# ZhengyiLuo/PHC

Hardware: AMD Instinct MI355X
Metric: env-steps/sec at 4096 humanoid envs per GPU (VecEnv.step incl. resets) (higher is better)
Workload: dtype f32

## Files before the change

### include/phc_amd.h

```cpp
#ifndef PHC_AMD_H
#define PHC_AMD_H
#include <stdint.h>

#ifdef __cplusplus
extern "C" {
#endif

#define PHC_ABI_VERSION 37
#define PHC_MAX_BODIES 64
#define PHC_EINVAL (-1)
#define PHC_EUNSUPPORTED (-2)
#define PHC_RESET_SUBLISTS 16
#define PHC_RESET_COUNT_STRIDE 32

typedef struct {
    int32_t num_bodies;
    int32_t num_dof;
    int32_t max_level;
    int32_t num_contact_pts;
    const int32_t* ints;
    const float* floats;
    int32_t num_collision_pairs;
    int32_t num_shapes;
    int32_t int_stride;
    int32_t float_stride;
    int32_t max_body_contact_pts;
} phc_model_t;

typedef struct {
    const float* frames;
    int64_t num_frames_total;
    int32_t frame_stride;
    int32_t num_bodies;
    int32_t num_motions;
    const float* motion_lengths;
    const float* motion_dt;
    const int64_t* motion_num_frames;
    const int64_t* length_starts;
    int32_t num_ext_bodies;
    int32_t dofs_per_joint;
} phc_motion_lib_t;

typedef struct {
    int32_t num_envs;
    float* root_states;
    float* dof_state;
    float* rigid_body_state;
    float* contact_force;
    float* dof_force;
    float* pd_target;
    float* force_sensor;
    const int32_t* env_shape;
    const float* pd_ref;
} phc_sim_state_t;

typedef struct {
    float sim_dt;
    int32_t substeps;
    int32_t control_freq_inv;
    float gravity_z;
    float contact_stiffness;
    float contact_damping;
    float friction;
    float friction_viscous;
    float angular_damping;
    float max_angular_velocity;
    float contact_offset;
    int32_t control_mode;
    float limit_stiffness;
    float limit_damping;
    int32_t self_collision;
    float self_stiffness_scale;
    float self_damping_ratio;
    int32_t lane_mapping;
    int32_t num_force_sensors;
    int32_t force_sensor_body[4];
    int32_t contact_model;
    int32_t contact_iterations;
    float contact_impedance;
    float max_depenetration_velocity;
    float bounce_threshold_velocity;
    float restitution;
    int32_t inertia_lag;
    int32_t force_average;
} phc_sim_params_t;

typedef struct {
    float dt;
    int32_t max_episode_length;
    float k_pos, k_rot, k_vel, k_ang_vel, w_pos, w_rot, w_vel, w_ang_vel;
    int32_t power_reward;
    float power_coefficient;
    int32_t enable_early_termination;
    int32_t use_mean_termination;
    int32_t disable_collision_check;
    int32_t local_root_obs, root_height_obs;
    int32_t num_track_bodies;
    const int32_t* track_slot;
    const int32_t* reset_mask;
    int32_t num_reset_bodies;
    int32_t first_reset_body;
    const float* termination_distances;
    int32_t num_key_bodies;
    const int32_t* key_body_ids;
    int32_t num_amp_joints;
    const int32_t* amp_joint_slot;
    int32_t num_amp_obs_steps;
    int32_t num_amp_obs_per_step;
    int32_t num_self_obs, num_task_obs;
    int32_t cycle_motion;
    int32_t zero_out_far;
    float close_distance;
    float far_distance;
    int32_t dofs_per_joint;
    int32_t num_ext_bodies;
    const int32_t* ext_parent;
    const float* ext_offset;
    int32_t obs_v;
    int32_t self_obs_v;
    int32_t num_force_sensors;
    int32_t amp_obs_v;
    int32_t remove_base_rot;
    int32_t num_self_obs_extra;
    int32_t num_amp_obs_extra;
    int32_t num_traj_samples;
    float traj_sample_timestep;
    int32_t track_body_reward;
    int32_t num_self_obs_hist;
    int32_t zero_out_far_train;
    int32_t zero_out_far_steps;
    int32_t cycle_motion_xp;
    const float* self_obs_extra;
    const float* amp_obs_extra;
    const float* amp_ref_table;
} phc_im_params_t;

typedef struct {
    int64_t* progress_buf;
    int64_t* reset_buf;
    int64_t* terminate_buf;
    float* rew_buf;
    float* reward_raw;
    float* obs_buf;
    float* amp_obs_in;
    float* amp_obs_out;
    const int64_t* sampled_motion_ids;
    float* motion_start_times;
    float* motion_start_times_offset;
    float* global_offset;
    float* ref_body_pos;
    float* ref_body_rot;
    float* ref_body_vel;
    float* ref_dof_pos;
    int32_t* cycle_counter;
    int32_t* recovery_counter;
    float* point_goal;
    const float* cycle_phase;
    int32_t* reset_list;
    int32_t* reset_count;
    int32_t reset_slot;
    int32_t reset_sublist_cap;
    float* body_state_hist;
    const float* offset_rand;
    const uint8_t* occl_mask;
    int64_t amp_env_stride;
    uint64_t* reset_rng_counter;
} phc_im_buffers_t;

int32_t phc_abi_version(void);

int32_t phc_motion_state(const phc_motion_lib_t* lib, int32_t n, const int64_t* motion_ids, const float* motion_times,
                         const float* offset, float* rg_pos , float* rb_rot ,
                         float* body_vel , float* body_ang_vel , float* dof_pos ,
                         float* dof_vel , int64_t* frame_idx0 , int64_t* frame_idx1 ,
                         float* blend , float* rg_pos_ext , float* rb_rot_ext , void* stream);

int32_t phc_sample_time_interval(const phc_motion_lib_t* lib, int32_t n, const int64_t* motion_ids, const float* phase,
                                 float* motion_times, void* stream);

int32_t phc_sim_step(const phc_model_t* model, const phc_sim_params_t* params, const phc_sim_state_t* sim,
                     const float* actions , const float* pd_action_offset , const float* pd_action_scale ,
                     const int32_t* freeze_mask , int32_t num_sim_calls, void* stream);

int32_t phc_sim_step_wrench(const phc_model_t* model, const phc_sim_params_t* params, const phc_sim_state_t* sim,
                            const float* actions , const float* pd_action_offset , const float* pd_action_scale ,
                            const int32_t* freeze_mask , int32_t num_sim_calls,
                            const float* ext_force , const float* ext_torque , int32_t wrench_sim_calls, void* stream);

int32_t phc_refresh_body_state(const phc_model_t* model, const phc_sim_state_t* sim, void* stream);

int32_t phc_refresh_body_state_indexed(const phc_model_t* model, const phc_sim_state_t* sim, int32_t num, const int64_t* env_ids,
                                       void* stream);

int32_t phc_im_post_physics(const phc_model_t* model, const phc_motion_lib_t* lib, const phc_im_params_t* prm,
                            const phc_sim_state_t* sim, const phc_im_buffers_t* buf, void* stream);

int32_t phc_amp_ref_table(const phc_model_t* model, const phc_motion_lib_t* lib, const phc_im_params_t* prm, int64_t num_frames,
                          const int64_t* next_frame , float* table , void* stream);

int32_t phc_im_reset(const phc_model_t* model, const phc_motion_lib_t* lib, const phc_im_params_t* prm,
                     const phc_sim_state_t* sim, const phc_im_buffers_t* buf, int32_t num_reset,
                     const int64_t* env_ids, const float* phase , int32_t start_at_zero, void* stream);

int32_t phc_im_is_plain(const phc_model_t* model, const phc_motion_lib_t* lib, const phc_im_params_t* prm, const phc_im_buffers_t* buf);
int32_t phc_task_force_generic(int32_t on);

int32_t phc_im_reset_done(const phc_model_t* model, const phc_motion_lib_t* lib, const phc_im_params_t* prm,
                          const phc_sim_state_t* sim, const phc_im_buffers_t* buf, uint64_t seed, uint64_t counter,
                          int32_t start_at_zero, void* stream);

int32_t phc_im_reset_from_state(const phc_model_t* model, const phc_motion_lib_t* lib, const phc_im_params_t* prm,
                                const phc_sim_state_t* sim, const phc_im_buffers_t* buf, int32_t num_reset,
                                const int64_t* env_ids, int32_t fill_history, void* stream);

int32_t phc_amp_obs_demo(const phc_model_t* model, const phc_motion_lib_t* lib, const phc_im_params_t* prm, int32_t n,
                         const int64_t* motion_ids, const float* motion_times0, float* amp_obs_demo , void* stream);

int32_t phc_gae(int32_t horizon, int32_t n, const float* fdones, const float* values, const float* rewards,
                const float* next_values, float gamma, float tau, float* advs, void* stream);

int32_t phc_fk(const phc_model_t* model, int64_t num_frames, const float* local_rot, const float* root_trans,
               float* global_rot, float* global_pos, void* stream);

int64_t phc_running_norm_workspace(int64_t rows, int32_t cols);
int32_t phc_running_norm(const float* x, const int64_t* row_index, int64_t rows, int32_t cols, const double* norm_mean, const double* norm_var, float epsilon,
                         float clamp, void* out, int32_t out_bf16, int32_t out_stride, double* run_mean, double* run_var, double* run_count,
                         double* workspace, void* stream);

int64_t phc_colsum_workspace(int64_t rows, int32_t cols);
int32_t phc_colsum_bf16(const void* x, int64_t rows, int32_t cols, float* out, float* workspace, void* stream);
int32_t phc_colsum_relu_bf16(const void* gy, const void* y, int64_t rows, int32_t cols, void* gm, float* out, float* workspace, void* stream);
#define PHC_COLSUM_MAX_JOBS 16
typedef struct {
    const float* partial;
    float* out;
    int32_t nchunks, cols, accumulate;
} phc_colsum_job_t;
int32_t phc_colsum_chunks(int64_t rows);
int32_t phc_linear1_chunks(int64_t rows);
int32_t phc_colsum_finish_batch(int32_t count, const phc_colsum_job_t* jobs , void* stream);
int32_t phc_sum_slabs_bf16(const void* part, int32_t slabs, int64_t n, float* out, int32_t accumulate, void* stream);
int32_t phc_split3_bf16(const float* x, int64_t ld_in, const float* gate, int64_t ld_gate, int64_t rows, int32_t cols, int64_t rows_pad, int32_t cols_pad,
                        const float* extra, int32_t extra_mode, void* out, int64_t row_stride, int64_t chunk_stride, int32_t order, void* stream);

int32_t phc_wgrad_bf16_slices(int64_t rows, int32_t n, int32_t k);
int64_t phc_wgrad_bf16_workspace(int64_t rows, int32_t n, int32_t k);
int32_t phc_wgrad_bf16(const void* gy, const void* y, const void* x, int64_t ld_x, int64_t rows, int32_t n, int32_t k, float* gw, int64_t ld_gw,
                       int32_t accumulate, void* gz, float* gb, int32_t gb_accumulate, void* workspace, void* stream);

int32_t phc_disc_bce(const void* logits, int32_t is_bf16, int32_t n_agent, int32_t n_demo, float scale, void* grad, float* stats,
                     void* stream);
int64_t phc_sumsq_workspace(void);
int32_t phc_weighted_sumsq(int32_t count, const void* const* tensors, const int64_t* sizes, const float* coefs, int32_t is_bf16, float* out,
                           double* workspace, void* stream);

int32_t phc_rollout_bookkeeping(const float* rewards, float reward_scale, const int64_t* dones, const int64_t* terminate, const float* reward_raw,
                                int32_t num_reward_terms, int64_t num_envs, float* exp_rewards, uint8_t* exp_dones, float* terminated_flags,
                                float* terminated_mask, float* reward_raw_acc, float* current_rewards, float* current_lengths, void* stream);

int32_t phc_policy_sample(const void* mu, const void* value, int32_t is_bf16, const float* logstd, const float* noise, const double* value_mean,
                          const double* value_var, float epsilon, const float* mask, int64_t num_envs, int32_t num_actions, float* actions, float* mus,
                          float* sigmas, float* neglogp, float* values, void* stream);

int64_t phc_linear1_workspace(int64_t rows, int32_t cols);
int32_t phc_linear1_forward(const void* x, const void* w, const void* b, int64_t rows, int32_t cols, void* y, void* stream);
int32_t phc_linear1_backward(const void* x, const void* w, const void* gy, int64_t rows, int32_t cols, void* gx, float* gw_gb,
                             float* workspace, void* stream);

int64_t phc_adam_workspace(void);
int32_t phc_adam_clip_step(float* param, float* grad, float* exp_avg, float* exp_avg_sq, int64_t n, float lr, float beta1, float beta2,
                           float eps, float weight_decay, int64_t step, float max_norm, double* workspace, float* grad_norm_out,
                           void* param_bf16, int64_t* step_device, void* stream);

typedef struct {
    float e_clip, critic_coef, entropy_coef, bounds_loss_coef;
    int32_t clip_value;
} phc_ppo_params_t;
int64_t phc_ppo_loss_workspace(void);
int32_t phc_ppo_loss(const void* mu, const void* value, int32_t is_bf16, const float* logstd, const float* actions, const float* old_neglogp,
                     const float* advantages, const float* returns, const float* old_values, const float* old_mu, const float* old_sigma,
                     const int64_t* row_index, int64_t batch, int32_t num_actions, const phc_ppo_params_t* prm, void* grad_mu, void* grad_value, float* stats,
                     double* workspace, void* stream);

#define PHC_RENDER_MAX_PIXELS (1 << 24)
#define PHC_RENDER_MAX_SHAPES 128
#define PHC_RENDER_MAX_MARKERS 128
#define PHC_RENDER_PALETTE 16
#define PHC_RENDER_MARKER_ID 1000
typedef struct {
    int32_t env;
    float eye[3], target[3], up[3];
    float fov_y;
} phc_camera_t;
typedef struct {
    int32_t num_envs, num_bodies;
    const float* body_state;
    const float* capsules;
    int32_t num_capsules;
    int32_t num_shape_blocks;
    int64_t capsule_stride;
    const int32_t* env_shape;
    const float* markers;
    int32_t num_markers;
    float marker_radius;
    float palette[PHC_RENDER_PALETTE][3];
    float marker_color[3];
    float ground_color[2][3];
    float sky_color[3];
    float light_dir[3];
    float ambient, diffuse;
} phc_render_scene_t;
int32_t phc_render(const phc_render_scene_t* scene , const phc_camera_t* cameras , int32_t views, int32_t width,
                   int32_t height, uint8_t* rgba, float* depth, int32_t* hit_id, void* stream);

typedef struct {
    int32_t num_envs, num_bodies;
    int32_t root_idx;
    int32_t step;
    int32_t bound;
    float dt;
    const float* rigid_body_state;
    const int64_t* progress_buf;
    const int64_t* terminate_buf;
    const int64_t* motion_ids;
    const float* motion_start_times;
    const float* motion_start_times_offset;
    const float* global_offset;
    const int32_t* clip_steps;
    float* history;
    double* sums;
    int32_t* count;
    int32_t* failed;
    int32_t* status;
    float* mpjpe_step;
    float* gt_out;
} phc_eval_args_t;
int32_t phc_eval_accumulate(const phc_motion_lib_t* lib, const phc_eval_args_t* args , void* stream);

typedef struct {
    int32_t num_envs, num_bodies;
    int32_t num_listed;
    int32_t pause_lo, pause_hi;
    int32_t duration;
    int32_t direction;
    float force_lo, force_hi;
    uint64_t key;
    int64_t env_offset;
    const int32_t* bodies;
    const int64_t* progress_buf;
    int32_t* remaining;
    int32_t* countdown;
    int32_t* body;
    int32_t* k;
    int32_t* started;
    float* force;
} phc_push_args_t;
int32_t phc_push_advance(const phc_push_args_t* args , void* stream);

#ifdef __cplusplus
}
#endif
#endif
```

### phc_amd/_lib.py

```python
import ctypes as C
import os

import torch

HERE = os.path.dirname(os.path.abspath(__file__))
LIB_PATH = os.environ.get("PHC_AMD_LIB") or os.path.join(HERE, "libphc_amd.so")

c_f = C.c_float
c_i32 = C.c_int32
c_i64 = C.c_int64
c_p = C.c_void_p


class Model(C.Structure):
    _fields_ = [("num_bodies", c_i32), ("num_dof", c_i32), ("max_level", c_i32), ("num_contact_pts", c_i32),
                ("ints", c_p), ("floats", c_p), ("num_collision_pairs", c_i32),
                ("num_shapes", c_i32), ("int_stride", c_i32), ("float_stride", c_i32), ("max_body_contact_pts", c_i32)]


class MotionLib(C.Structure):
    _fields_ = [("frames", c_p), ("num_frames_total", c_i64), ("frame_stride", c_i32), ("num_bodies", c_i32),
                ("num_motions", c_i32), ("motion_lengths", c_p), ("motion_dt", c_p), ("motion_num_frames", c_p),
                ("length_starts", c_p), ("num_ext_bodies", c_i32), ("dofs_per_joint", c_i32)]


class SimState(C.Structure):
    _fields_ = [("num_envs", c_i32), ("root_states", c_p), ("dof_state", c_p), ("rigid_body_state", c_p),
                ("contact_force", c_p), ("dof_force", c_p), ("pd_target", c_p), ("force_sensor", c_p), ("env_shape", c_p), ("pd_ref", c_p)]


class SimParams(C.Structure):
    _fields_ = [("sim_dt", c_f), ("substeps", c_i32), ("control_freq_inv", c_i32), ("gravity_z", c_f),
                ("contact_stiffness", c_f), ("contact_damping", c_f), ("friction", c_f), ("friction_viscous", c_f),
                ("angular_damping", c_f), ("max_angular_velocity", c_f), ("contact_offset", c_f),
                ("control_mode", c_i32), ("limit_stiffness", c_f), ("limit_damping", c_f),
                ("self_collision", c_i32), ("self_stiffness_scale", c_f), ("self_damping_ratio", c_f), ("lane_mapping", c_i32),
                ("num_force_sensors", c_i32), ("force_sensor_body", c_i32 * 4),
                ("contact_model", c_i32), ("contact_iterations", c_i32), ("contact_impedance", c_f), ("max_depenetration_velocity", c_f),
                ("bounce_threshold_velocity", c_f), ("restitution", c_f), ("inertia_lag", c_i32), ("force_average", c_i32)]


class ColsumJob(C.Structure):
    _fields_ = [("partial", c_p), ("out", c_p), ("nchunks", c_i32), ("cols", c_i32), ("accumulate", c_i32)]


class ImParams(C.Structure):
    _fields_ = [("dt", c_f), ("max_episode_length", c_i32),
                ("k_pos", c_f), ("k_rot", c_f), ("k_vel", c_f), ("k_ang_vel", c_f),
                ("w_pos", c_f), ("w_rot", c_f), ("w_vel", c_f), ("w_ang_vel", c_f),
                ("power_reward", c_i32), ("power_coefficient", c_f),
                ("enable_early_termination", c_i32), ("use_mean_termination", c_i32), ("disable_collision_check", c_i32),
                ("local_root_obs", c_i32), ("root_height_obs", c_i32),
                ("num_track_bodies", c_i32), ("track_slot", c_p), ("reset_mask", c_p), ("num_reset_bodies", c_i32), ("first_reset_body", c_i32),
                ("termination_distances", c_p),
                ("num_key_bodies", c_i32), ("key_body_ids", c_p),
                ("num_amp_joints", c_i32), ("amp_joint_slot", c_p),
                ("num_amp_obs_steps", c_i32), ("num_amp_obs_per_step", c_i32),
                ("num_self_obs", c_i32), ("num_task_obs", c_i32),
                ("cycle_motion", c_i32), ("zero_out_far", c_i32), ("close_distance", c_f), ("far_distance", c_f),
                ("dofs_per_joint", c_i32), ("num_ext_bodies", c_i32), ("ext_parent", c_p), ("ext_offset", c_p), ("obs_v", c_i32),
                ("self_obs_v", c_i32), ("num_force_sensors", c_i32), ("amp_obs_v", c_i32),
                ("remove_base_rot", c_i32), ("num_self_obs_extra", c_i32), ("num_amp_obs_extra", c_i32),
                ("num_traj_samples", c_i32), ("traj_sample_timestep", c_f), ("track_body_reward", c_i32), ("num_self_obs_hist", c_i32), ("zero_out_far_train", c_i32), ("zero_out_far_steps", c_i32), ("cycle_motion_xp", c_i32),
                ("self_obs_extra", c_p), ("amp_obs_extra", c_p), ("amp_ref_table", c_p)]


class ImBuffers(C.Structure):
    _fields_ = [("progress_buf", c_p), ("reset_buf", c_p), ("terminate_buf", c_p), ("rew_buf", c_p), ("reward_raw", c_p),
                ("obs_buf", c_p), ("amp_obs_in", c_p), ("amp_obs_out", c_p), ("sampled_motion_ids", c_p),
                ("motion_start_times", c_p), ("motion_start_times_offset", c_p), ("global_offset", c_p),
                ("ref_body_pos", c_p), ("ref_body_rot", c_p), ("ref_body_vel", c_p), ("ref_dof_pos", c_p),
                ("cycle_counter", c_p), ("recovery_counter", c_p), ("point_goal", c_p), ("cycle_phase", c_p),
                ("reset_list", c_p), ("reset_count", c_p), ("reset_slot", c_i32), ("reset_sublist_cap", c_i32), ("body_state_hist", c_p), ("offset_rand", c_p), ("occl_mask", c_p), ("amp_env_stride", C.c_int64), ("reset_rng_counter", c_p)]


class PpoParams(C.Structure):
    _fields_ = [("e_clip", c_f), ("critic_coef", c_f), ("entropy_coef", c_f), ("bounds_loss_coef", c_f), ("clip_value", c_i32)]


RENDER_PALETTE = 16
RENDER_MARKER_ID = 1000
RENDER_MAX_PIXELS = 1 << 24
RENDER_MAX_SHAPES = 128
RENDER_MAX_MARKERS = 128


class Camera(C.Structure):
    _fields_ = [("env", c_i32), ("eye", c_f * 3), ("target", c_f * 3), ("up", c_f * 3), ("fov_y", c_f)]


class RenderScene(C.Structure):
    _fields_ = [("num_envs", c_i32), ("num_bodies", c_i32), ("body_state", c_p), ("capsules", c_p), ("num_capsules", c_i32),
                ("num_shape_blocks", c_i32), ("capsule_stride", c_i64), ("env_shape", c_p), ("markers", c_p), ("num_markers", c_i32),
                ("marker_radius", c_f), ("palette", (c_f * 3) * RENDER_PALETTE), ("marker_color", c_f * 3), ("ground_color", (c_f * 3) * 2),
                ("sky_color", c_f * 3), ("light_dir", c_f * 3), ("ambient", c_f), ("diffuse", c_f)]


class EvalArgs(C.Structure):
    _fields_ = [("num_envs", c_i32), ("num_bodies", c_i32), ("root_idx", c_i32), ("step", c_i32), ("bound", c_i32), ("dt", c_f),
                ("rigid_body_state", c_p), ("progress_buf", c_p), ("terminate_buf", c_p), ("motion_ids", c_p), ("motion_start_times", c_p),
                ("motion_start_times_offset", c_p), ("global_offset", c_p), ("clip_steps", c_p), ("history", c_p), ("sums", c_p), ("count", c_p),
                ("failed", c_p), ("status", c_p), ("mpjpe_step", c_p), ("gt_out", c_p)]


class PushArgs(C.Structure):
    _fields_ = [("num_envs", c_i32), ("num_bodies", c_i32), ("num_listed", c_i32), ("pause_lo", c_i32), ("pause_hi", c_i32), ("duration", c_i32),
                ("direction", c_i32), ("force_lo", c_f), ("force_hi", c_f), ("key", C.c_uint64), ("env_offset", c_i64), ("bodies", c_p),
                ("progress_buf", c_p), ("remaining", c_p), ("countdown", c_p), ("body", c_p), ("k", c_p), ("started", c_p), ("force", c_p)]


P = C.POINTER
_SIGNATURES = {
    "phc_abi_version": ([], c_i32),
    "phc_motion_state": ([P(MotionLib), c_i32] + [c_p] * 15, c_i32),
    "phc_sample_time_interval": ([P(MotionLib), c_i32, c_p, c_p, c_p, c_p], c_i32),
    "phc_sim_step": ([P(Model), P(SimParams), P(SimState), c_p, c_p, c_p, c_p, c_i32, c_p], c_i32),
    "phc_sim_step_wrench": ([P(Model), P(SimParams), P(SimState), c_p, c_p, c_p, c_p, c_i32, c_p, c_p, c_i32, c_p], c_i32),
    "phc_refresh_body_state": ([P(Model), P(SimState), c_p], c_i32),
    "phc_im_post_physics": ([P(Model), P(MotionLib), P(ImParams), P(SimState), P(ImBuffers), c_p], c_i32),
    "phc_amp_ref_table": ([P(Model), P(MotionLib), P(ImParams), c_i64, c_p, c_p, c_p], c_i32),
    "phc_im_reset": ([P(Model), P(MotionLib), P(ImParams), P(SimState), P(ImBuffers), c_i32, c_p, c_p, c_i32, c_p], c_i32),
    "phc_im_reset_done": ([P(Model), P(MotionLib), P(ImParams), P(SimState), P(ImBuffers), C.c_uint64, C.c_uint64, c_i32, c_p], c_i32),
    "phc_im_reset_from_state": ([P(Model), P(MotionLib), P(ImParams), P(SimState), P(ImBuffers), c_i32, c_p, c_i32, c_p], c_i32),
    "phc_refresh_body_state_indexed": ([P(Model), P(SimState), c_i32, c_p, c_p], c_i32),
    "phc_amp_obs_demo": ([P(Model), P(MotionLib), P(ImParams), c_i32, c_p, c_p, c_p, c_p], c_i32),
    "phc_gae": ([c_i32, c_i32, c_p, c_p, c_p, c_p, c_f, c_f, c_p, c_p], c_i32),
    "phc_fk": ([P(Model), c_i64, c_p, c_p, c_p, c_p, c_p], c_i32),
    "phc_running_norm_workspace": ([c_i64, c_i32], c_i64),
    "phc_running_norm": ([c_p, c_p, c_i64, c_i32, c_p, c_p, c_f, c_f, c_p, c_i32, c_i32, c_p, c_p, c_p, c_p, c_p], c_i32),
    "phc_colsum_workspace": ([c_i64, c_i32], c_i64),
    "phc_colsum_bf16": ([c_p, c_i64, c_i32, c_p, c_p, c_p], c_i32),
    "phc_colsum_relu_bf16": ([c_p, c_p, c_i64, c_i32, c_p, c_p, c_p, c_p], c_i32),
    "phc_sum_slabs_bf16": ([c_p, c_i32, c_i64, c_p, c_i32, c_p], c_i32),
    "phc_wgrad_bf16_slices": ([c_i64, c_i32, c_i32], c_i32),
    "phc_wgrad_bf16_workspace": ([c_i64, c_i32, c_i32], c_i64),
    "phc_wgrad_bf16": ([c_p, c_p, c_p, c_i64, c_i64, c_i32, c_i32, c_p, c_i64, c_i32, c_p, c_p, c_i32, c_p, c_p], c_i32),
    "phc_split3_bf16": ([c_p, c_i64, c_p, c_i64, c_i64, c_i32, c_i64, c_i32, c_p, c_i32, c_p, c_i64, c_i64, c_i32, c_p], c_i32),
    "phc_colsum_chunks": ([c_i64], c_i32),
    "phc_linear1_chunks": ([c_i64], c_i32),
    "phc_colsum_finish_batch": ([c_i32, P(ColsumJob), c_p], c_i32),
    "phc_rollout_bookkeeping": ([c_p, c_f, c_p, c_p, c_p, c_i32, c_i64, c_p, c_p, c_p, c_p, c_p, c_p, c_p, c_p], c_i32),
    "phc_disc_bce": ([c_p, c_i32, c_i32, c_i32, c_f, c_p, c_p, c_p], c_i32),
    "phc_sumsq_workspace": ([], c_i64),
    "phc_weighted_sumsq": ([c_i32, c_p, c_p, c_p, c_i32, c_p, c_p, c_p], c_i32),
    "phc_policy_sample": ([c_p, c_p, c_i32, c_p, c_p, c_p, c_p, c_f, c_p, c_i64, c_i32, c_p, c_p, c_p, c_p, c_p, c_p], c_i32),
    "phc_linear1_workspace": ([c_i64, c_i32], c_i64),
    "phc_linear1_forward": ([c_p, c_p, c_p, c_i64, c_i32, c_p, c_p], c_i32),
    "phc_linear1_backward": ([c_p, c_p, c_p, c_i64, c_i32, c_p, c_p, c_p, c_p], c_i32),
    "phc_adam_workspace": ([], c_i64),
    "phc_adam_clip_step": ([c_p, c_p, c_p, c_p, c_i64, c_f, c_f, c_f, c_f, c_f, c_i64, c_f, c_p, c_p, c_p, c_p, c_p], c_i32),
    "phc_ppo_loss_workspace": ([], c_i64),
    "phc_ppo_loss": ([c_p, c_p, c_i32] + [c_p] * 9 + [c_i64, c_i32, P(PpoParams), c_p, c_p, c_p, c_p, c_p], c_i32),
    "phc_render": ([P(RenderScene), P(Camera), c_i32, c_i32, c_i32, c_p, c_p, c_p, c_p], c_i32),
    "phc_eval_accumulate": ([P(MotionLib), P(EvalArgs), c_p], c_i32),
    "phc_push_advance": ([P(PushArgs), c_p], c_i32),
}
_OPTIONAL_SIGNATURES = {
    "phc_im_is_plain": ([P(Model), P(MotionLib), P(ImParams), P(ImBuffers)], c_i32),
    "phc_task_force_generic": ([c_i32], c_i32),
}
EXPORTED_SYMBOLS = tuple(_SIGNATURES) + tuple(_OPTIONAL_SIGNATURES)

_lib = None


def load():
    global _lib
    if _lib is not None:
        return _lib
    if not os.path.exists(LIB_PATH):
        raise ImportError(f"{LIB_PATH} not found: build the HIP extension first "
                          "(python -m phc_amd.build or __graft_entry__.build()); there is no CPU fallback")
    lib = C.CDLL(LIB_PATH)
    for name, (argtypes, restype) in _SIGNATURES.items():
        fn = getattr(lib, name)
        fn.argtypes = argtypes
        fn.restype = restype
    for name, (argtypes, restype) in _OPTIONAL_SIGNATURES.items():
        fn = getattr(lib, name, None)
        if fn is not None:
            fn.argtypes = argtypes
            fn.restype = restype
    if lib.phc_abi_version() != 37:
        raise ImportError("libphc_amd.so ABI version mismatch")
    _lib = lib
    return lib


class PhcError(RuntimeError):
    pass


def check(rc, what):
    if rc != 0:
        kind = {-1: "invalid argument", -2: "unsupported configuration"}.get(rc, f"hipError {rc}")
        raise PhcError(f"{what} failed: {kind}")
```

### phc_amd/abi.py

```python
import ctypes as C

import numpy as np

from . import _lib as L

MAX_BODIES = 64
NUM_INT_TABLES = 21


def ptr(x):
    if x is None:
        return None
    if isinstance(x, np.ndarray):
        assert x.flags["C_CONTIGUOUS"], "numpy array must be C-contiguous"
        return x.ctypes.data
    assert x.is_contiguous(), "tensor must be contiguous"
    return x.data_ptr()


def model_struct(ints, floats, num_bodies, num_dof, max_level, num_contact_pts, num_shapes=1):
    m = L.Model()
    m.num_shapes = int(num_shapes)
    if num_shapes > 1:
        assert ints.ndim == 2 and floats.ndim == 2 and ints.shape[0] == floats.shape[0] == num_shapes
        m.int_stride, m.float_stride = int(ints.shape[1]), int(floats.shape[1])
        m.num_collision_pairs = int(ints[:, 4 + NUM_INT_TABLES * MAX_BODIES].max())
    else:
        m.num_collision_pairs = int(ints.reshape(-1)[4 + NUM_INT_TABLES * MAX_BODIES])
    m.num_bodies, m.num_dof, m.max_level, m.num_contact_pts = num_bodies, num_dof, max_level, num_contact_pts
    per_body = ints.reshape(max(1, int(num_shapes)), -1)[:, 4 + 9 * MAX_BODIES:4 + 10 * MAX_BODIES]
    m.max_body_contact_pts = int(per_body.max())
    m.ints, m.floats = ptr(ints), ptr(floats)
    return m


def motion_lib_struct(frames, frame_stride, num_bodies, motion_lengths, motion_dt, motion_num_frames, length_starts,
                      num_ext_bodies=0, dofs_per_joint=3):
    s = L.MotionLib()
    s.num_ext_bodies, s.dofs_per_joint = int(num_ext_bodies), int(dofs_per_joint)
    s.frames = ptr(frames)
    s.num_frames_total = int(frames.shape[0])
    s.frame_stride = int(frame_stride)
    s.num_bodies = int(num_bodies)
    s.num_motions = int(motion_lengths.shape[0])
    s.motion_lengths, s.motion_dt = ptr(motion_lengths), ptr(motion_dt)
    s.motion_num_frames, s.length_starts = ptr(motion_num_frames), ptr(length_starts)
    return s


def sim_state_struct(num_envs, root_states, dof_state, rigid_body_state, contact_force, dof_force, pd_target, force_sensor=None, env_shape=None, pd_ref=None):
    s = L.SimState()
    s.pd_ref = ptr(pd_ref)
    s.force_sensor = ptr(force_sensor)
    s.env_shape = ptr(env_shape)
    s.num_envs = int(num_envs)
    s.root_states, s.dof_state, s.rigid_body_state = ptr(root_states), ptr(dof_state), ptr(rigid_body_state)
    s.contact_force, s.dof_force, s.pd_target = ptr(contact_force), ptr(dof_force), ptr(pd_target)
    return s


def sim_params_struct(sim_dt=1 / 60, substeps=2, control_freq_inv=2, gravity_z=-9.81, contact_stiffness=1.0e5,
                      contact_damping=1.0e3, friction=1.0, friction_viscous=2.0e3, angular_damping=0.01,
                      max_angular_velocity=100.0, contact_offset=0.02, control_mode=0, limit_stiffness=0.0, limit_damping=0.0, lane_mapping=0,
                      self_collision=0, self_stiffness_scale=0.25, self_damping_ratio=0.5, force_sensor_bodies=(), contact_model=0,
                      contact_iterations=4, contact_impedance=1.0e5, max_depenetration_velocity=10.0, bounce_threshold_velocity=0.2, restitution=0.0,
                      inertia_lag=0, force_average=0):
    p = L.SimParams()
    if isinstance(contact_model, str) and contact_model not in ("penalty", "tgs", "rigid"):
        raise ValueError(f"solver.contact must be 'penalty' or 'tgs' (alias 'rigid'), not {contact_model!r}")
    p.contact_model = {"penalty": 0, "tgs": 1, "rigid": 1}.get(contact_model, contact_model)
    p.inertia_lag, p.force_average = int(bool(inertia_lag)), int(bool(force_average))
    if p.contact_model == 1 and p.inertia_lag:
        raise ValueError("solver.inertia_lag needs the penalty contact model (the rigid model re-solves every sub-step with fresh impedances)")
    if p.contact_model == 1 and int(contact_iterations) < 2:
        raise ValueError("solver.contact_iterations must be >= 2 for the rigid contact model")
    p.contact_iterations, p.contact_impedance = int(contact_iterations), float(contact_impedance)
    p.max_depenetration_velocity, p.bounce_threshold_velocity, p.restitution = float(max_depenetration_velocity), float(bounce_threshold_velocity), float(restitution)
    assert len(force_sensor_bodies) <= 4, "at most 4 force sensors"
    p.num_force_sensors = len(force_sensor_bodies)
    for i, b in enumerate(force_sensor_bodies):
        p.force_sensor_body[i] = int(b)
    p.sim_dt, p.substeps, p.control_freq_inv, p.gravity_z = sim_dt, substeps, control_freq_inv, gravity_z
    p.contact_stiffness, p.contact_damping, p.friction, p.friction_viscous = contact_stiffness, contact_damping, friction, friction_viscous
    p.angular_damping, p.max_angular_velocity, p.contact_offset = angular_damping, max_angular_velocity, contact_offset
    p.control_mode, p.limit_stiffness, p.limit_damping = int(control_mode), float(limit_stiffness), float(limit_damping)
    p.lane_mapping = int(lane_mapping)
    p.self_collision, p.self_stiffness_scale, p.self_damping_ratio = int(self_collision), float(self_stiffness_scale), float(self_damping_ratio)
    return p


def frame_stride_for(num_bodies, num_ext_bodies=0, dofs_per_joint=3):
    nbe = num_bodies + num_ext_bodies
    n = nbe * 7 + num_bodies * 6 + ((num_bodies - 1) * 2 if dofs_per_joint == 1 else num_bodies * 4 + (num_bodies - 1) * 3)
    return (n + 3) // 4 * 4


def pack_frames(gts, grs, gvs, gavs, lrs, dvs, xp=np, gts_ext=None, grs_ext=None, dof_pos=None):
    F_, nb = gts.shape[0], gts.shape[1]
    ne = 0 if gts_ext is None else gts_ext.shape[1]
    dpj = 1 if dof_pos is not None else 3
    stride = frame_stride_for(nb, ne, dpj)
    if xp is np:
        out = np.zeros((F_, stride), dtype=np.float32)
        cat = lambda a, b: np.concatenate([a, b], axis=1)
    else:
        out = xp.zeros((F_, stride), dtype=xp.float32, device=gts.device)
        cat = lambda a, b: xp.cat([a, b], dim=1)
    pos = gts if ne == 0 else cat(gts, gts_ext)
    rot = grs if ne == 0 else cat(grs, grs_ext)
    o = 0
    fields = [(pos, (nb + ne) * 3), (rot, (nb + ne) * 4), (gvs, nb * 3), (gavs, nb * 3)]
    fields += [(dof_pos, nb - 1), (dvs, nb - 1)] if dpj == 1 else [(lrs, nb * 4), (dvs, (nb - 1) * 3)]
    for arr, w in fields:
        out[:, o:o + w] = arr.reshape(F_, w)
        o += w
    return out


def im_params_struct(dt, max_episode_length, reward_specs, power_reward, power_coefficient, enable_early_termination,
                     use_mean_termination, disable_collision_check, local_root_obs, root_height_obs, num_track_bodies,
                     track_slot, reset_mask, num_reset_bodies, first_reset_body, termination_distances, num_key_bodies, key_body_ids,
                     num_amp_joints, amp_joint_slot, num_amp_obs_steps, num_amp_obs_per_step, num_self_obs, num_task_obs,
                     cycle_motion=False, zero_out_far=False, close_distance=0.25, far_distance=3.0,
                     dofs_per_joint=3, ext_parent=None, ext_offset=None, obs_v=6, self_obs_v=1, num_force_sensors=0, amp_obs_v=1,
                     remove_base_rot=False, self_obs_extra=None, amp_obs_extra=None, zero_out_far_train=False, zero_out_far_steps=90,
                     cycle_motion_xp=False, num_self_obs_hist=0, track_body_reward=False, num_traj_samples=1, traj_sample_timestep=1 / 30, amp_ref_table=None):
    p = L.ImParams()
    p.remove_base_rot = int(bool(remove_base_rot))
    p.num_self_obs_hist = int(num_self_obs_hist)
    p.track_body_reward = int(bool(track_body_reward))
    p.num_traj_samples, p.traj_sample_timestep = int(num_traj_samples), float(np.float32(traj_sample_timestep))
    p.zero_out_far_train, p.zero_out_far_steps, p.cycle_motion_xp = int(bool(zero_out_far_train)), int(zero_out_far_steps), int(bool(cycle_motion_xp))
    p.num_self_obs_extra = 0 if self_obs_extra is None else int(self_obs_extra.shape[1])
    p.num_amp_obs_extra = 0 if amp_obs_extra is None else int(amp_obs_extra.shape[1])
    p.self_obs_extra, p.amp_obs_extra = ptr(self_obs_extra), ptr(amp_obs_extra)
    p.amp_ref_table = ptr(amp_ref_table)
    p.amp_obs_v = int(amp_obs_v)
    p.obs_v = int(obs_v)
    p.self_obs_v, p.num_force_sensors = int(self_obs_v), int(num_force_sensors)
    p.dofs_per_joint = int(dofs_per_joint)
    p.num_ext_bodies = 0 if ext_parent is None else int(ext_parent.shape[0])
    p.ext_parent, p.ext_offset = ptr(ext_parent), ptr(ext_offset)
    p.dt = float(np.float32(dt))
    p.max_episode_length = int(max_episode_length)
    for k in ("k_pos", "k_rot", "k_vel", "k_ang_vel", "w_pos", "w_rot", "w_vel", "w_ang_vel"):
        setattr(p, k, float(reward_specs[k]))
    p.power_reward, p.power_coefficient = int(bool(power_reward)), float(power_coefficient)
    p.enable_early_termination = int(bool(enable_early_termination))
    p.use_mean_termination = int(bool(use_mean_termination))
    p.disable_collision_check = int(bool(disable_collision_check))
    p.local_root_obs, p.root_height_obs = int(bool(local_root_obs)), int(bool(root_height_obs))
    p.num_track_bodies, p.track_slot = int(num_track_bodies), ptr(track_slot)
    p.reset_mask, p.num_reset_bodies = ptr(reset_mask), int(num_reset_bodies)
    p.first_reset_body = int(first_reset_body)
    p.termination_distances = ptr(termination_distances)
    p.num_key_bodies, p.key_body_ids = int(num_key_bodies), ptr(key_body_ids)
    p.num_amp_joints, p.amp_joint_slot = int(num_amp_joints), ptr(amp_joint_slot)
    p.num_amp_obs_steps, p.num_amp_obs_per_step = int(num_amp_obs_steps), int(num_amp_obs_per_step)
    p.num_self_obs, p.num_task_obs = int(num_self_obs), int(num_task_obs)
    p.cycle_motion, p.zero_out_far = int(bool(cycle_motion)), int(bool(zero_out_far))
    p.close_distance, p.far_distance = float(close_distance), float(far_distance)
    return p


RESET_SUBLISTS = 16
RESET_COUNT_STRIDE = 32


def reset_sublist_cap(num_envs):
    blocks = (num_envs + 7) // 8
    return 8 * ((blocks + RESET_SUBLISTS - 1) // RESET_SUBLISTS)


def im_buffers_struct(progress_buf, reset_buf, terminate_buf, rew_buf, reward_raw, obs_buf, amp_obs_in, amp_obs_out,
                      sampled_motion_ids, motion_start_times, motion_start_times_offset, global_offset,
                      ref_body_pos=None, ref_body_rot=None, ref_body_vel=None, ref_dof_pos=None,
                      cycle_counter=None, recovery_counter=None, point_goal=None, cycle_phase=None, reset_list=None, reset_count=None,
                      reset_slot=0, offset_rand=None, body_state_hist=None, occl_mask=None, amp_env_stride=0, reset_rng_counter=None):
    b = L.ImBuffers()
    b.amp_env_stride = int(amp_env_stride)
    b.reset_rng_counter = ptr(reset_rng_counter)
    b.occl_mask = ptr(occl_mask)
    b.offset_rand = ptr(offset_rand)
    b.body_state_hist = ptr(body_state_hist)
    b.reset_list, b.reset_count, b.reset_slot = ptr(reset_list), ptr(reset_count), int(reset_slot)
    b.reset_sublist_cap = 0 if reset_list is None else int(reset_list.shape[0]) // RESET_SUBLISTS
    b.progress_buf, b.reset_buf, b.terminate_buf = ptr(progress_buf), ptr(reset_buf), ptr(terminate_buf)
    b.rew_buf, b.reward_raw, b.obs_buf = ptr(rew_buf), ptr(reward_raw), ptr(obs_buf)
    first = lambda t: t.ctypes.data if isinstance(t, np.ndarray) else t.data_ptr()
    b.amp_obs_in, b.amp_obs_out = (ptr(t) if amp_env_stride == 0 else first(t) for t in (amp_obs_in, amp_obs_out))
    b.sampled_motion_ids = ptr(sampled_motion_ids)
    b.motion_start_times, b.motion_start_times_offset = ptr(motion_start_times), ptr(motion_start_times_offset)
    b.global_offset = ptr(global_offset)
    b.ref_body_pos, b.ref_body_rot, b.ref_body_vel, b.ref_dof_pos = ptr(ref_body_pos), ptr(ref_body_rot), ptr(ref_body_vel), ptr(ref_dof_pos)
    b.cycle_counter, b.recovery_counter = ptr(cycle_counter), ptr(recovery_counter)
    b.point_goal, b.cycle_phase = ptr(point_goal), ptr(cycle_phase)
    return b


def task_index_tables(model, track_bodies, reset_bodies, key_bodies, amp_remove_names=("L_Hand", "R_Hand", "L_Toe", "R_Toe"),
                      has_dof_subset=True):
    MB = MAX_BODIES
    names = model.body_names
    track_slot = np.full(MB, -1, dtype=np.int32)
    for s, n in enumerate(track_bodies):
        track_slot[names.index(n)] = s
    reset_mask = np.zeros(MB, dtype=np.int32)
    for n in reset_bodies:
        reset_mask[names.index(n)] = 1
    key_ids = np.array([names.index(n) for n in key_bodies], dtype=np.int32)
    amp_slot = np.full(MB, -1, dtype=np.int32)
    s = 0
    for j in range(1, len(names)):
        if (not has_dof_subset) or names[j] not in amp_remove_names:
            amp_slot[j] = s
            s += 1
    return track_slot, reset_mask, key_ids, amp_slot, s
```

### phc_amd/build.py

```python
import os
import shutil
import subprocess
import sys

HERE = os.path.dirname(os.path.abspath(__file__))
CSRC = os.path.join(HERE, "csrc")
LIB = os.path.join(HERE, "libphc_amd.so")
SOURCES = {"phc_kernels.hip": ["-fno-slp-vectorize", "-ffp-contract=off"], "phc_kernels_plain.hip": ["-fno-slp-vectorize", "-ffp-contract=off"], "phc_sim.hip": ["-ffast-math", "-fno-slp-vectorize"],
           "phc_sim_wrench.hip": ["-ffast-math", "-fno-slp-vectorize"],
           "phc_learn.hip": ["-ffp-contract=off"], "phc_gemm.hip": ["-ffp-contract=off"], "phc_render.hip": [], "phc_eval.hip": ["-ffp-contract=off"],
           "phc_push.hip": ["-ffp-contract=off"]}
HEADERS = ["phc_math.h", "phc_task.h", "phc_im.h", "phc_im_check.h", "phc_im_plain.h", "phc_task_kernel.h", "phc_aba.h", "phc_sim_kernel.h", "phc_sim_check.h", "phc_eval.h", "phc_group.h", "phc_rng.h", "phc_push.h", os.path.join("..", "..", "include", "phc_amd.h")]


def _hipcc():
    for c in (os.environ.get("HIPCC"), shutil.which("hipcc"), "/opt/rocm/bin/hipcc"):
        if c and os.path.exists(c):
            return c
    raise RuntimeError("hipcc not found: the HIP extension cannot be built")


def needs_build():
    if not os.path.exists(LIB):
        return True
    t = os.path.getmtime(LIB)
    return any(os.path.getmtime(os.path.join(CSRC, f)) > t for f in list(SOURCES) + HEADERS)


def build(force=False, verbose=False):
    if not force and not needs_build():
        return LIB
    hipcc = _hipcc()
    common = ["--offload-arch=gfx950", "-O3", "-std=c++17", "-fPIC", "-Wno-comment"]
    objs = []
    os.makedirs(os.path.join(HERE, "_obj"), exist_ok=True)
    for src, extra in SOURCES.items():
        obj = os.path.join(HERE, "_obj", src.replace(".hip", ".o"))
        cmd = [hipcc, *common, *extra, "-c", os.path.join(CSRC, src), "-o", obj]
        if verbose:
            print(" ".join(cmd))
        r = subprocess.run(cmd, capture_output=True, text=True)
        if r.returncode != 0:
            raise RuntimeError(f"hipcc failed on {src}:\n" + r.stdout + r.stderr)
        objs.append(obj)
    cmd = [hipcc, "--offload-arch=gfx950", "-shared", "-fPIC", *objs, "-o", LIB]
    if verbose:
        print(" ".join(cmd))
    r = subprocess.run(cmd, capture_output=True, text=True)
    if r.returncode != 0:
        raise RuntimeError("hipcc link failed:\n" + r.stdout + r.stderr)
    return LIB


if __name__ == "__main__":
    print(build(force="--force" in sys.argv, verbose=True))
```

### phc_amd/csrc/phc_aba.h

```cpp
#pragma once
#include "phc_math.h"
#include "../../include/phc_amd.h"

namespace phc {

#define PHC_XCH_STRIDE 28
#define PHC_BODY_FLOATS 56
#define PHC_CAP_STRIDE 20
#define PHC_SC_FSCALE 1024.0f
#define PHC_SC_NSCALE 4096.0f
#define PHC_JT_SPHERICAL 1
#define PHC_JT_REVOLUTE 2
#define PHC_NTAB 21

#if defined(PHC_CP_MASK32)
typedef uint32_t CpMask;
#define PHC_CP_CTZ(x) __builtin_ctz(x)
#else
typedef uint64_t CpMask;
#define PHC_CP_CTZ(x) __builtin_ctzll(x)
#endif
#define PHC_CP_BITS ((int)(8 * sizeof(CpMask)))

struct Sym3 { float xx, xy, xz, yy, yz, zz; };

PHC_HD V3 sym_mul(const Sym3& s, V3 v) {
    return v3(s.xx * v.x + s.xy * v.y + s.xz * v.z, s.xy * v.x + s.yy * v.y + s.yz * v.z, s.xz * v.x + s.yz * v.y + s.zz * v.z);
}
PHC_HD Sym3 sym_inv(const Sym3& s) {
    float c00 = s.yy * s.zz - s.yz * s.yz;
    float c01 = s.xz * s.yz - s.xy * s.zz;
    float c02 = s.xy * s.yz - s.xz * s.yy;
    float det = s.xx * c00 + s.xy * c01 + s.xz * c02;
    float id = 1.0f / det;
    Sym3 r;
    r.xx = c00 * id; r.xy = c01 * id; r.xz = c02 * id;
    r.yy = (s.xx * s.zz - s.xz * s.xz) * id;
    r.yz = (s.xy * s.xz - s.xx * s.yz) * id;
    r.zz = (s.xx * s.yy - s.xy * s.xy) * id;
    return r;
}
PHC_HD Sym3 rot_diag(const M3& R, V3 d) {
    Sym3 s;
    const float* m = R.m;
    s.xx = m[0] * m[0] * d.x + m[1] * m[1] * d.y + m[2] * m[2] * d.z;
    s.xy = m[0] * m[3] * d.x + m[1] * m[4] * d.y + m[2] * m[5] * d.z;
    s.xz = m[0] * m[6] * d.x + m[1] * m[7] * d.y + m[2] * m[8] * d.z;
    s.yy = m[3] * m[3] * d.x + m[4] * m[4] * d.y + m[5] * m[5] * d.z;
    s.yz = m[3] * m[6] * d.x + m[4] * m[7] * d.y + m[5] * m[8] * d.z;
    s.zz = m[6] * m[6] * d.x + m[7] * m[7] * d.y + m[8] * m[8] * d.z;
    return s;
}
PHC_HD Sym3 rot_sym(const M3& R, const Sym3& S) {
    float t[9];
    for (int i = 0; i < 3; ++i) {
        float a = R.m[3 * i], b = R.m[3 * i + 1], c = R.m[3 * i + 2];
        t[3 * i + 0] = a * S.xx + b * S.xy + c * S.xz;
        t[3 * i + 1] = a * S.xy + b * S.yy + c * S.yz;
        t[3 * i + 2] = a * S.xz + b * S.yz + c * S.zz;
    }
    Sym3 r;
    r.xx = t[0] * R.m[0] + t[1] * R.m[1] + t[2] * R.m[2];
    r.xy = t[0] * R.m[3] + t[1] * R.m[4] + t[2] * R.m[5];
    r.xz = t[0] * R.m[6] + t[1] * R.m[7] + t[2] * R.m[8];
    r.yy = t[3] * R.m[3] + t[4] * R.m[4] + t[5] * R.m[5];
    r.yz = t[3] * R.m[6] + t[4] * R.m[7] + t[5] * R.m[8];
    r.zz = t[6] * R.m[6] + t[7] * R.m[7] + t[8] * R.m[8];
    return r;
}

struct Inertia6 { Sym3 A; float B[9]; Sym3 C; };
struct Force6 { V3 n, f; };

PHC_HD V3 B_mul(const float* B, V3 v) {
    return v3(B[0] * v.x + B[1] * v.y + B[2] * v.z, B[3] * v.x + B[4] * v.y + B[5] * v.z, B[6] * v.x + B[7] * v.y + B[8] * v.z);
}
PHC_HD V3 Bt_mul(const float* B, V3 v) {
    return v3(B[0] * v.x + B[3] * v.y + B[6] * v.z, B[1] * v.x + B[4] * v.y + B[7] * v.z, B[2] * v.x + B[5] * v.y + B[8] * v.z);
}

struct AbaLane {
    int parent, level, dof_start;
    int sparent, slevel, nchild, child[3];
    int anchors;
    int jsrc;
    int bsrc;
    V3 r_local;
    float mass, cp_bound; int cp_range;
    Q4 q;
    V3 wj;
    V3 target;
    Q4 Q; V3 p, w, v;
    V3 rw, cw, ca;
    Inertia6 IA; Force6 pA;
    Sym3 Di; V3 u;
    Sym3 Dw;
    float diso;
    V3 tau_w;
    V3 aw;
    V3 tau_local;
    V3 dimp;
    V3 arm;
    V3 fcontact;
    V3 axis;
    Q4 qrest;
    float th, thd;
    float tau_hold;
    V3 fself, nself;
    V3 cap_a, cap_b; float cap_r, cap_m; int cap_owner;
    V3 acc_w, acc_v;
    uint32_t c_active, c_removed;
    CpMask c_touch;
};

PHC_HD phc_model_t model_for_env(phc_model_t m, const phc_sim_state_t& s, int64_t env) {
    if (m.num_shapes > 1 && s.env_shape != nullptr && env < s.num_envs) {
        const int sh = s.env_shape[env];
        m.ints += (int64_t)sh * m.int_stride;
        m.floats += (int64_t)sh * m.float_stride;
    }
    return m;
}
PHC_HD const float* model_body(const phc_model_t& m, int j) { return m.floats + j * PHC_BODY_FLOATS; }
PHC_HD int model_tab(const phc_model_t& m, int table, int j) { return m.ints[4 + table * PHC_MAX_BODIES + j]; }

PHC_HD int model_solver_depth(const phc_model_t& m, bool reroot) { return reroot ? model_tab(m, 11, 2) : m.max_level; }
struct SolverRef { V3 off, mc; Sym3 Io; };
PHC_HD SolverRef model_solver_ref(const float* f, bool reroot) {
    SolverRef r;
    const int o = reroot ? 47 : 4;
    r.off = reroot ? v3(f[44], f[45], f[46]) : v3(0.f, 0.f, 0.f);
    r.mc = v3(f[o], f[o + 1], f[o + 2]);
    r.Io.xx = f[o + 3]; r.Io.xy = f[o + 4]; r.Io.xz = f[o + 5]; r.Io.yy = f[o + 6]; r.Io.yz = f[o + 7]; r.Io.zz = f[o + 8];
    return r;
}

PHC_HD void aba_load_model(AbaLane& L, const phc_model_t& m, int j, bool reroot = true) {
    L.parent = model_tab(m, 0, j); L.level = model_tab(m, 1, j);
    L.dof_start = model_tab(m, 3, j);
    L.anchors = model_tab(m, 20, j);
    if (reroot) {
        L.sparent = model_tab(m, 13, j); L.slevel = model_tab(m, 14, j);
        L.child[0] = model_tab(m, 15, j); L.child[1] = model_tab(m, 16, j); L.child[2] = model_tab(m, 17, j);
        L.nchild = model_tab(m, 18, j);
        const int js = model_tab(m, 19, j);
        L.jsrc = (js & 0xff) - 1; L.bsrc = ((js >> 8) & 0xff) - 1;
    } else {
        L.sparent = L.parent; L.slevel = L.level;
        L.child[0] = model_tab(m, 4, j); L.child[1] = model_tab(m, 5, j); L.child[2] = model_tab(m, 6, j);
        L.nchild = model_tab(m, 7, j);
        L.jsrc = j > 0 ? j : -1; L.bsrc = -1;
    }
    L.rw = L.cw = L.ca = v3(0.f, 0.f, 0.f);
    const float* f = model_body(m, j);
    L.r_local = v3(f[0], f[1], f[2]);
    L.mass = f[3]; L.cp_bound = f[34];
    L.cp_range = model_tab(m, 8, j) | (model_tab(m, 9, j) << 16);
    L.arm = v3(f[19], f[20], f[21]);
    L.fself = L.nself = v3(0.f, 0.f, 0.f);
    L.cap_a = v3(f[36], f[37], f[38]); L.cap_b = v3(f[39], f[40], f[41]); L.cap_r = f[42]; L.cap_m = f[3]; L.cap_owner = j;
}
template <int JT, bool RIGID = false>
PHC_HD void aba_body_init(AbaLane& L, const phc_model_t& m, const phc_sim_params_t& prm, float dt, int j, bool new_sim_call, bool reroot = true, int pass = 0, bool lag = false,
                          bool ext_on = false, V3 ext_f = V3(), V3 ext_t = V3());

PHC_HD void aba_load_model_rev(AbaLane& L, const phc_model_t& m, int j) {
    const float* f = model_body(m, j);
    L.axis = v3(f[25], f[26], f[27]);
    L.qrest = q4(f[28], f[29], f[30], f[31]);
    L.tau_hold = 0.f;
}
PHC_HD Q4 rev_joint_quat(const AbaLane& L) { return quat_mul16(L.qrest, quat_from_rotvec(L.axis * L.th)); }

template <int JT>
PHC_HD void aba_load_state(AbaLane& L, const phc_sim_state_t& s, int nd, int64_t env, int j, bool load_target = true) {
    if (j == 0) {
        const float* r = s.root_states + env * 13;
        L.p = v3(r[0], r[1], r[2]); L.q = quat_normalize(q4(r[3], r[4], r[5], r[6]));
        L.v = v3(r[7], r[8], r[9]); L.w = v3(r[10], r[11], r[12]);
        L.wj = v3(0.f, 0.f, 0.f); L.target = v3(0.f, 0.f, 0.f);
        if (JT == PHC_JT_REVOLUTE) { L.th = L.thd = 0.f; }
    } else if (JT == PHC_JT_REVOLUTE) {
        const float* d = s.dof_state + (env * nd + L.dof_start) * 2;
        L.th = d[0]; L.thd = d[1];
        L.q = rev_joint_quat(L);
        L.wj = L.axis * L.thd;
        L.target = load_target ? v3(s.pd_target[env * nd + L.dof_start], 0.f, 0.f) : v3(0.f, 0.f, 0.f);
    } else {
        const float* d = s.dof_state + (env * nd + L.dof_start) * 2;
        L.q = quat_from_rotvec(v3(d[0], d[2], d[4]));
        L.wj = v3(d[1], d[3], d[5]);
        const float* t = s.pd_target + env * nd + L.dof_start;
        L.target = load_target ? v3(t[0], t[1], t[2]) : v3(0.f, 0.f, 0.f);
    }
}

struct Xch {
    float* base;
    static constexpr int bs = PHC_XCH_STRIDE;
    static constexpr int es = 1;
};
PHC_HD float* xslot(const Xch& x, int body) { return x.base + body * Xch::bs; }

PHC_HD void aba_kinematics_from_parent(AbaLane& L, Q4 Qp, V3 pp, V3 wp, V3 vp) {
    const V3 r = quat_rotate(Qp, L.r_local);
    L.p = pp + r;
    L.Q = quat_mul16(Qp, L.q);
    V3 wJw = quat_rotate(L.Q, L.wj);
    L.w = wp + wJw;
    L.v = vp + cross(wp, r);
}
PHC_HD void aba_velocity_products(AbaLane& L, const phc_model_t& m, int j, const Xch& x, bool reroot, const float* offs = nullptr) {
    if (L.slevel <= 0) { L.rw = L.cw = L.ca = v3(0.f, 0.f, 0.f); return; }
    constexpr int es = Xch::es;
    const float* ps = xslot(x, L.sparent);
    const V3 pp = v3(ps[10 * es], ps[11 * es], ps[12 * es]), wp = v3(ps[13 * es], ps[14 * es], ps[15 * es]);
    L.rw = L.p - pp;
    if (reroot) {
        const float* f = offs ? offs + 3 * j : model_body(m, j) + 44;
        const float* fp = offs ? offs + 3 * L.sparent : model_body(m, L.sparent) + 44;
        L.rw = L.rw + quat_rotate(L.Q, v3(f[0], f[1], f[2]))
                    - quat_rotate(q4(ps[6 * es], ps[7 * es], ps[8 * es], ps[9 * es]), v3(fp[0], fp[1], fp[2]));
    }
    L.cw = cross(wp, L.w - wp);
    L.ca = cross(wp, cross(wp, L.rw));
}
PHC_HD void aba_write_kin(const AbaLane& L, float* s, int es, int o) {
    s[(o + 0) * es] = L.Q.x; s[(o + 1) * es] = L.Q.y; s[(o + 2) * es] = L.Q.z; s[(o + 3) * es] = L.Q.w;
    s[(o + 4) * es] = L.p.x; s[(o + 5) * es] = L.p.y; s[(o + 6) * es] = L.p.z;
    s[(o + 7) * es] = L.w.x; s[(o + 8) * es] = L.w.y; s[(o + 9) * es] = L.w.z;
    s[(o + 10) * es] = L.v.x; s[(o + 11) * es] = L.v.y; s[(o + 12) * es] = L.v.z;
}

PHC_HD void aba_fk_level(AbaLane& L, int level, int j, const Xch& x) {
    if (L.level != level) return;
    constexpr int es = Xch::es;
    if (level == 0) {
        L.Q = L.q;
    } else {
        const float* ps = xslot(x, L.parent);
        aba_kinematics_from_parent(L, q4(ps[6 * es], ps[7 * es], ps[8 * es], ps[9 * es]), v3(ps[10 * es], ps[11 * es], ps[12 * es]),
                                   v3(ps[13 * es], ps[14 * es], ps[15 * es]), v3(ps[16 * es], ps[17 * es], ps[18 * es]));
    }
    aba_write_kin(L, xslot(x, j), es, 6);
}

PHC_HD int model_jump_steps(const phc_model_t& m) { return model_tab(m, 11, 4); }
PHC_HD void aba_fk_jump_begin(AbaLane& L, int j, const Xch& x) {
    if (L.level < 0) return;
    if (L.level == 0) { L.Q = L.q; }
    else { L.Q = L.q; L.p = L.r_local; L.w = quat_rotate(L.q, L.wj); L.v = v3(0.f, 0.f, 0.f); }
    aba_write_kin(L, xslot(x, j), Xch::es, 6);
}
PHC_HD void aba_fk_jump_step(AbaLane& L, int k, const Xch& x) {
    if (L.level < 0) return;
    const int a = (L.anchors >> (8 * k)) & 0xff;
    if (a == 0xff) return;
    constexpr int es = Xch::es;
    const float* s = xslot(x, a);
    const Q4 Qa = q4(s[6 * es], s[7 * es], s[8 * es], s[9 * es]);
    const V3 pa = v3(s[10 * es], s[11 * es], s[12 * es]), wa = v3(s[13 * es], s[14 * es], s[15 * es]), va = v3(s[16 * es], s[17 * es], s[18 * es]);
    const M3 Ra = quat_to_mat(Qa);
    const V3 r = mat_mul(Ra, L.p);
    L.v = va + cross(wa, r) + mat_mul(Ra, L.v);
    L.w = wa + mat_mul(Ra, L.w);
    L.p = pa + r;
    L.Q = quat_mul16(Qa, L.Q);
}

PHC_HD void aba_add_point_contact(AbaLane& L, V3 arm, V3 F0, float c1, float c3) {
    L.pA.n -= cross(arm, F0);
    L.pA.f -= F0;
    const float ax = arm.x, ay = arm.y, az = arm.z;
    L.IA.A.xx += az * az * c1 + ay * ay * c3;
    L.IA.A.yy += az * az * c1 + ax * ax * c3;
    L.IA.A.zz += (ax * ax + ay * ay) * c1;
    L.IA.A.xy -= ax * ay * c3;
    L.IA.A.xz -= ax * az * c1;
    L.IA.A.yz -= ay * az * c1;
    L.IA.B[1] += -az * c1; L.IA.B[2] += ay * c3;
    L.IA.B[3] += az * c1;  L.IA.B[5] += -ax * c3;
    L.IA.B[6] += -ay * c1; L.IA.B[7] += ax * c1;
    L.IA.C.xx += c1; L.IA.C.yy += c1; L.IA.C.zz += c3;
}

PHC_HD float rigid_point_velocity_target(const phc_sim_params_t& prm, float dt, float depth, float un_now) {
    float vt = depth > 0.f ? fminf(depth / dt, prm.max_depenetration_velocity) : depth / dt;
    if (prm.restitution > 0.f && -un_now > prm.bounce_threshold_velocity) vt = fmaxf(vt, -prm.restitution * un_now);
    return vt;
}
struct RigidPoint { V3 arm, uc, un, cc; float depth, lam; };
PHC_HD bool rigid_point(const AbaLane& L, const phc_sim_params_t& prm, float dt, const M3& R, V3 so, const float* cpk, bool predicted, RigidPoint* o) {
    V3 arm = mat_mul(R, v3(cpk[0], cpk[1], cpk[2]));
    const float rad = cpk[3];
    o->depth = rad - (L.p.z + arm.z);
    if (o->depth <= -prm.contact_offset) return false;
    arm.z -= rad;
    o->uc = L.v + cross(L.w, arm);
    o->arm = arm - so;
    o->cc = cross(L.w, cross(L.w, o->arm));
    o->un = predicted ? o->uc + (L.acc_v + cross(L.acc_w, o->arm) + o->cc) * dt : o->uc;
    o->lam = prm.contact_impedance * (rigid_point_velocity_target(prm, dt, o->depth, o->uc.z) - o->un.z);
    return true;
}
PHC_HD float rigid_point_ct(const phc_sim_params_t& prm, const RigidPoint& q) {
    const float us = sqrtf(q.uc.x * q.uc.x + q.uc.y * q.uc.y), up = sqrtf(q.un.x * q.un.x + q.un.y * q.un.y);
    return fminf(prm.contact_impedance, prm.friction * q.lam / (fmaxf(us, up) + 1e-9f));
}
PHC_HD void aba_ground_contact_rigid(AbaLane& L, const phc_sim_params_t& prm, float dt, const M3& R, V3 so, const float* f, const float* cp,
                                     int cp_total, int pass) {
    const float c = prm.contact_impedance;
    if (pass == 0) L.c_active = L.c_removed = 0u;
    uint32_t act = 0u;
    const int cp_count = (L.p.z < f[34] + prm.contact_offset) ? cp_total : 0;
    for (int k = 0; k < cp_count; ++k) {
        RigidPoint q;
        if (!rigid_point(L, prm, dt, R, so, cp + 4 * k, pass > 0, &q)) continue;
        const uint32_t bit = k < 32 ? 1u << k : 0u;
        if (q.lam <= 0.f) { L.c_removed |= L.c_active & bit; continue; }
        if (L.c_removed & bit) continue;
        act |= bit;
        const float vt = rigid_point_velocity_target(prm, dt, q.depth, q.uc.z);
        const float ct = rigid_point_ct(prm, q);
        const V3 F0 = v3(-ct * q.uc.x - dt * ct * q.cc.x, -ct * q.uc.y - dt * ct * q.cc.y, c * (vt - q.uc.z) - dt * c * q.cc.z);
        aba_add_point_contact(L, q.arm, F0, dt * ct, dt * c);
    }
    L.c_active = act;
}
PHC_HD void aba_ground_force_rigid(const AbaLane& L, const phc_sim_params_t& prm, float dt, const M3& R, V3 so, const float* f, const float* cp,
                                   int cp_total, V3* Fout, V3* Nout) {
    V3 F = v3(0.f, 0.f, 0.f), N = v3(0.f, 0.f, 0.f);
    const int cp_count = (L.p.z < f[34] + prm.contact_offset) ? cp_total : 0;
    for (int k = 0; k < cp_count; ++k) {
        RigidPoint q;
        if (!rigid_point(L, prm, dt, R, so, cp + 4 * k, true, &q) || q.lam <= 0.f) continue;
        if (k < 32 && !((L.c_active >> k) & 1u)) continue;
        const float ct = rigid_point_ct(prm, q);
        const V3 Fk = v3(-ct * q.un.x, -ct * q.un.y, q.lam);
        F += Fk;
        N += cross(q.arm + so, Fk);
    }
    *Fout = F; *Nout = N;
}

template <int JT, bool RIGID>
PHC_HD constexpr bool aba_batched_constants() { return !RIGID && JT == PHC_JT_SPHERICAL; }

PHC_HD CpMask cp_touching_serial(const M3& R, float pz, const float* cp, int n) {
    CpMask touching = 0;
#if defined(__HIP_DEVICE_COMPILE__)
#pragma unroll 8
#endif
    for (int k = 0; k < n; ++k) {
        const float az = R.m[6] * cp[4 * k] + R.m[7] * cp[4 * k + 1] + R.m[8] * cp[4 * k + 2];
        if (cp[4 * k + 3] - (pz + az) > 0.f) touching |= (CpMask)1 << k;
    }
    return touching;
}
PHC_HD CpMask cp_touching_batched(const M3& R, float pz, const float* cp, int n) {
    constexpr int CG = 8;
    CpMask touching = 0;
    auto group = [&](int k0) {
        float c[CG][4];
        for (int i = 0; i < CG; ++i) {
            const int k = k0 + i < n ? k0 + i : n - 1;
            for (int e = 0; e < 4; ++e) c[i][e] = cp[4 * k + e];
        }
        for (int i = 0; i < CG; ++i) {
            const float az = R.m[6] * c[i][0] + R.m[7] * c[i][1] + R.m[8] * c[i][2];
            const bool t = (c[i][3] - (pz + az) > 0.f) & (k0 + i < n);
            touching |= (CpMask)(t ? 1 : 0) << (k0 + i);
        }
    };
    if (n > 0) group(0);
    for (int k0 = CG; k0 < n; k0 += CG) group(k0);
    return touching;
}

PHC_HD void aba_add_wrench(AbaLane& L, V3 mc, float mass, V3 F, V3 T) {
    L.pA.f -= F;
    L.pA.n -= T + cross(mc, F) * (1.0f / mass);
}

template <int JT, bool RIGID>
PHC_HD void aba_body_init(AbaLane& L, const phc_model_t& m, const phc_sim_params_t& prm, float dt, int j, bool new_sim_call,
                          const float* f, int cp_start, int cp_total, bool reroot, int pass, bool lag = false,
                          bool ext_on = false, V3 ext_f = V3(), V3 ext_t = V3()) {
    constexpr bool BATCH = aba_batched_constants<JT, RIGID>();
    const float mass = BATCH ? L.mass : f[3];
    const SolverRef sr = model_solver_ref(f, reroot);
    float fd[12];
    if (BATCH) for (int k = 0; k < 12; ++k) fd[k] = f[13 + k];
    M3 R = quat_to_mat(L.Q);
    const float* cp = m.floats + PHC_MAX_BODIES * PHC_BODY_FLOATS + cp_start * 4;
    int cp_count = 0;
    CpMask touching = 0;
    if (BATCH) {
        cp_count = (L.p.z < L.cp_bound) ? cp_total : 0;
        touching = cp_touching_batched(R, L.p.z, cp, cp_count < PHC_CP_BITS ? cp_count : PHC_CP_BITS);
    }
    Sym3 Io = rot_sym(R, sr.Io);
    V3 mc = mat_mul(R, sr.mc);
    const V3 so = mat_mul(R, sr.off);
    if (!lag) {
        L.IA.A = Io;
        L.IA.B[0] = 0.f;   L.IA.B[1] = -mc.z; L.IA.B[2] = mc.y;
        L.IA.B[3] = mc.z;  L.IA.B[4] = 0.f;   L.IA.B[5] = -mc.x;
        L.IA.B[6] = -mc.y; L.IA.B[7] = mc.x;  L.IA.B[8] = 0.f;
        L.IA.C.xx = L.IA.C.yy = L.IA.C.zz = mass; L.IA.C.xy = L.IA.C.xz = L.IA.C.yz = 0.f;
    }
    V3 g = v3(0.f, 0.f, prm.gravity_z);
    L.pA.n = cross(L.w, sym_mul(Io, L.w)) - cross(mc, g);
    L.pA.f = cross(L.w, cross(L.w, mc)) - g * mass;
    if (ext_on) aba_add_wrench(L, mc, mass, ext_f, ext_t);
    L.fcontact = v3(0.f, 0.f, 0.f);
    if (RIGID) {
        aba_ground_contact_rigid(L, prm, dt, R, so, f, cp, cp_total, pass);
    } else {
    const float cn = prm.contact_stiffness * dt + prm.contact_damping;
    if (!BATCH) {
        cp_count = (L.p.z < f[34]) ? cp_total : 0;
        touching = cp_touching_serial(R, L.p.z, cp, cp_count < PHC_CP_BITS ? cp_count : PHC_CP_BITS);
    }
    if (lag) touching &= L.c_touch;
    struct Cp4 { float x, y, z, r; };
    auto cp_load = [&](int k) { Cp4 c; c.x = cp[4 * k]; c.y = cp[4 * k + 1]; c.z = cp[4 * k + 2]; c.r = cp[4 * k + 3]; return c; };
    auto cp_point = [&](const Cp4& c) -> bool {
        V3 arm = mat_mul(R, v3(c.x, c.y, c.z));
        const float rad = c.r;
        const float depth = rad - (L.p.z + arm.z);
        if (depth <= 0.f) return false;
        arm.z -= rad;
        const V3 uc = L.v + cross(L.w, arm);
        arm = arm - so;
        const float fn0 = prm.contact_stiffness * depth - cn * uc.z;
        if (fn0 <= 0.f) return false;
        const float ut = sqrtf(uc.x * uc.x + uc.y * uc.y);
        const float ct = fminf(prm.friction_viscous, prm.friction * fn0 / (ut + 1e-6f));
        const V3 cc = cross(L.w, cross(L.w, arm));
        const V3 F0 = v3(-ct * uc.x - dt * ct * cc.x, -ct * uc.y - dt * ct * cc.y, fn0 - dt * cn * cc.z);
        L.fcontact += F0;
        if (lag) { L.pA.n -= cross(arm, F0); L.pA.f -= F0; }
        else aba_add_point_contact(L, arm, F0, dt * ct, dt * cn);
        return true;
    };
    CpMask pushed = 0;
    if (touching != 0) {
        CpMask rest = touching;
        int k = PHC_CP_CTZ(rest);
        rest &= rest - 1;
        Cp4 cur = cp_load(k);
        while (true) {
            const bool more = rest != 0;
            const int kn = more ? PHC_CP_CTZ(rest) : k;
            rest &= rest - 1;
            const Cp4 nxt = cp_load(kn);
            if (cp_point(cur)) pushed |= (CpMask)1 << k;
            if (!more) break;
            k = kn; cur = nxt;
        }
    }
    if (!lag) {
        for (int k = PHC_CP_BITS; k < cp_count; ++k) cp_point(cp_load(k));
        L.c_touch = pushed;
    }
    }
    L.fcontact += L.fself;
    L.pA.n -= L.nself - cross(so, L.fself);
    L.pA.f -= L.fself;
    if (RIGID && pass > 0) return;
    if (JT == PHC_JT_REVOLUTE) {
        if (L.level > 0) {
            const float kp = f[13], kd = f[16], eff = f[22];
            float tau, d;
            if (prm.control_mode == 1) {
                if (new_sim_call) L.tau_hold = fminf(fmaxf(kp * (L.target.x - L.th) - kd * L.thd, -eff), eff);
                tau = L.tau_hold;
                d = 0.f;
            } else if (prm.control_mode == 2) {
                if (new_sim_call) {
                    const float sp = kp * (L.target.x - L.th);
                    const float t0 = sp - kd * L.thd;
                    L.tau_hold = (fabsf(t0) >= eff) ? (t0 > 0.f ? eff : -eff) : sp;
                    L.target.y = (fabsf(t0) >= eff) ? 1.f : 0.f;
                }
                if (L.target.y != 0.f) { tau = L.tau_hold; d = 0.f; }
                else { tau = L.tau_hold - kd * L.thd; d = dt * kd; }
            } else {
                tau = fminf(fmaxf(kp * (L.target.x - L.th), -eff), eff) - (kd + dt * kp) * L.thd;
                d = dt * kd + dt * dt * kp;
            }
            if (prm.limit_stiffness > 0.f) {
                const float lo = f[32], hi = f[33];
                const float e = L.th < lo ? lo - L.th : (L.th > hi ? hi - L.th : 0.f);
                if (e != 0.f) {
                    if (!lag || L.target.z != 0.f) {
                        tau += prm.limit_stiffness * e - (prm.limit_damping + dt * prm.limit_stiffness) * L.thd;
                        d += dt * prm.limit_damping + dt * dt * prm.limit_stiffness;
                    } else {
                        tau += prm.limit_stiffness * e;
                    }
                }
                if (!lag) L.target.z = e != 0.f ? 1.f : 0.f;
            }
            L.tau_local = L.axis * tau;
            L.dimp = v3(d, 0.f, 0.f);
            L.aw = mat_mul(R, L.axis);
            L.tau_w = L.aw * tau;
        }
        return;
    }
    if (L.level > 0) {
        Q4 qt = quat_from_rotvec(L.target);
        V3 err = quat_to_rotvec(quat_mul16(quat_conjugate(L.q), qt));
        const float* fg = BATCH ? fd : f + 13;
        const V3 kp = v3(fg[0], fg[1], fg[2]), kd = v3(fg[3], fg[4], fg[5]), eff = v3(fg[9], fg[10], fg[11]);
        V3 sp = v3(fminf(fmaxf(kp.x * err.x, -eff.x), eff.x), fminf(fmaxf(kp.y * err.y, -eff.y), eff.y), fminf(fmaxf(kp.z * err.z, -eff.z), eff.z));
        V3 tau = v3(sp.x - (kd.x + dt * kp.x) * L.wj.x, sp.y - (kd.y + dt * kp.y) * L.wj.y, sp.z - (kd.z + dt * kp.z) * L.wj.z);
        V3 d = v3(dt * kd.x + dt * dt * kp.x, dt * kd.y + dt * dt * kp.y, dt * kd.z + dt * dt * kp.z);
        L.tau_local = tau;
        L.dimp = d;
        const V3 dd = d + v3(fg[6], fg[7], fg[8]);
        if (dd.x == dd.y && dd.y == dd.z) { L.diso = dd.x; }
        else { L.diso = -1.f; if (!lag) L.Dw = rot_diag(R, dd); }
        L.tau_w = mat_mul(R, tau);
    }
}

template <int JT, bool RIGID>
PHC_HD void aba_body_init(AbaLane& L, const phc_model_t& m, const phc_sim_params_t& prm, float dt, int j, bool new_sim_call, bool reroot, int pass, bool lag,
                          bool ext_on, V3 ext_f, V3 ext_t) {
    aba_body_init<JT, RIGID>(L, m, prm, dt, j, new_sim_call, model_body(m, j), model_tab(m, 8, j), model_tab(m, 9, j), reroot, pass, lag, ext_on, ext_f, ext_t);
}
PHC_HD void aba_publish_contact_rigid(AbaLane& L, const phc_model_t& m, const phc_sim_params_t& prm, const phc_sim_state_t& s, float dt,
                                      int64_t env, int j, bool reroot) {
    const float* f = model_body(m, j);
    const M3 R = quat_to_mat(L.Q);
    const V3 so = mat_mul(R, model_solver_ref(f, reroot).off);
    V3 F, N;
    aba_ground_force_rigid(L, prm, dt, R, so, f, m.floats + PHC_MAX_BODIES * PHC_BODY_FLOATS + model_tab(m, 8, j) * 4, model_tab(m, 9, j), &F, &N);
    L.fcontact = F + L.fself;
    if (s.force_sensor != nullptr)
        for (int k = 0; k < prm.num_force_sensors; ++k)
            if (prm.force_sensor_body[k] == j) {
                const V3 Fl = mat_tmul(R, F), Nl = mat_tmul(R, N);
                float* o = s.force_sensor + (env * prm.num_force_sensors + k) * 6;
                o[0] = Fl.x; o[1] = Fl.y; o[2] = Fl.z; o[3] = Nl.x; o[4] = Nl.y; o[5] = Nl.z;
            }
}

PHC_HD void seg_seg_closest(V3 p1, V3 q1, V3 p2, V3 q2, V3* c1, V3* c2) {
    const V3 d1 = q1 - p1, d2 = q2 - p2, r = p1 - p2;
    const float a = dot(d1, d1), e = dot(d2, d2), f = dot(d2, r);
    const float EPS = 1e-10f;
    float s = 0.f, t = 0.f;
    if (a <= EPS && e <= EPS) {
    } else if (a <= EPS) {
        t = fminf(fmaxf(f / e, 0.f), 1.f);
    } else {
        const float c = dot(d1, r);
        if (e <= EPS) {
            s = fminf(fmaxf(-c / a, 0.f), 1.f);
        } else {
            const float b = dot(d1, d2), denom = a * e - b * b;
            s = denom > 1e-7f * a * e ? fminf(fmaxf((b * f - c * e) / denom, 0.f), 1.f) : 0.f;
            t = (b * s + f) / e;
            if (t < 0.f) { t = 0.f; s = fminf(fmaxf(-c / a, 0.f), 1.f); }
            else if (t > 1.f) { t = 1.f; s = fminf(fmaxf((b - c) / a, 0.f), 1.f); }
        }
    }
    *c1 = p1 + d1 * s;
    *c2 = p2 + d2 * t;
}
PHC_HD int model_num_extra_shapes(const phc_model_t& m) { return model_tab(m, 11, 5); }
PHC_HD const float* model_extra_shape(const phc_model_t& m, int e) { return m.floats + PHC_MAX_BODIES * PHC_BODY_FLOATS + m.ints[3] * 4 + e * 8; }
PHC_HD int model_num_pairs(const phc_model_t& m) { return m.ints[4 + PHC_NTAB * PHC_MAX_BODIES]; }
PHC_HD int model_pair(const phc_model_t& m, int q) { return m.ints[4 + PHC_NTAB * PHC_MAX_BODIES + 1 + q]; }
PHC_HD void sc_atomic_add(int32_t* p, int32_t v) {
#if defined(__HIP_DEVICE_COMPILE__)
    atomicAdd(p, v);
#else
    *p += v;
#endif
}
PHC_HD void cap_write(float* cap, V3 a, V3 b, float radius, float mass, int owner) {
    const V3 mid = (a + b) * 0.5f;
    cap[0] = mid.x; cap[1] = mid.y; cap[2] = mid.z; cap[3] = 0.5f * norm(b - a) + radius;
    cap[4] = a.x; cap[5] = a.y; cap[6] = a.z; cap[7] = radius;
    cap[8] = b.x; cap[9] = b.y; cap[10] = b.z; cap[11] = mass;
    int32_t* acc = reinterpret_cast<int32_t*>(cap + 12);
    for (int k = 0; k < 6; ++k) acc[k] = 0;
    acc[6] = owner;
}
PHC_HD void aba_load_extra_shape(AbaLane& L, const phc_model_t& m, int e) {
    const float* r = model_extra_shape(m, e);
    L.cap_a = v3(r[0], r[1], r[2]); L.cap_b = v3(r[3], r[4], r[5]); L.cap_r = r[6]; L.cap_owner = (int)r[7];
    L.cap_m = model_body(m, L.cap_owner)[3];
}
PHC_HD void aba_publish_shape(const AbaLane& L, int s, const Xch& x, float* caps) {
    constexpr int es = Xch::es;
    const float* k = xslot(x, L.cap_owner);
    const M3 R = quat_to_mat(q4(k[6 * es], k[7 * es], k[8 * es], k[9 * es]));
    const V3 p = v3(k[10 * es], k[11 * es], k[12 * es]);
    cap_write(caps + PHC_CAP_STRIDE * s, p + mat_mul(R, L.cap_a), p + mat_mul(R, L.cap_b), L.cap_r, L.cap_m, L.cap_owner);
}
#define PHC_SC_SKIP_MARGIN 0.12f
PHC_HD int aba_pair_broad(int i, int k, const float* caps) {
    const float* ci = caps + PHC_CAP_STRIDE * i;
    const float* ck = caps + PHC_CAP_STRIDE * k;
    const V3 dm = v3(ci[0] - ck[0], ci[1] - ck[1], ci[2] - ck[2]);
    const float R = ci[3] + ck[3];
    const float d2 = dot(dm, dm);
    if (d2 <= R * R) return 0;
    return d2 > (R + PHC_SC_SKIP_MARGIN) * (R + PHC_SC_SKIP_MARGIN) ? 2 : 1;
}
PHC_HD bool aba_pair_narrow(const phc_sim_params_t& prm, float dt, int i, int k, const Xch& x, float* caps) {
    const float* ci = caps + PHC_CAP_STRIDE * i;
    const float* ck = caps + PHC_CAP_STRIDE * k;
    const V3 a1 = v3(ci[4], ci[5], ci[6]), b1 = v3(ci[8], ci[9], ci[10]), a2 = v3(ck[4], ck[5], ck[6]), b2 = v3(ck[8], ck[9], ck[10]);
    const float r1 = ci[7], m1 = ci[11], r2 = ck[7], m2 = ck[11];
    V3 c1, c2;
    seg_seg_closest(a1, b1, a2, b2, &c1, &c2);
    V3 n = c1 - c2;
    const float dist = norm(n), pen = r1 + r2 - dist;
    if (pen <= 0.f) return pen < -PHC_SC_SKIP_MARGIN;
    n = dist > 1e-6f ? n * (1.0f / dist) : v3(0.f, 0.f, 1.f);
    const V3 cp = c2 + n * (r2 - 0.5f * pen);
    constexpr int es = Xch::es;
    const int oi = reinterpret_cast<const int32_t*>(ci + 12)[6], ok = reinterpret_cast<const int32_t*>(ck + 12)[6];
    const float* si = xslot(x, oi);
    const float* sk = xslot(x, ok);
    const V3 pi = v3(si[10 * es], si[11 * es], si[12 * es]), wi = v3(si[13 * es], si[14 * es], si[15 * es]), vi = v3(si[16 * es], si[17 * es], si[18 * es]);
    const V3 pk = v3(sk[10 * es], sk[11 * es], sk[12 * es]), wk = v3(sk[13 * es], sk[14 * es], sk[15 * es]), vk = v3(sk[16 * es], sk[17 * es], sk[18 * es]);
    const V3 vrel = (vi + cross(wi, cp - pi)) - (vk + cross(wk, cp - pk));
    const float mu = m1 * m2 / (m1 + m2);
    const float kk = prm.self_stiffness_scale * mu / (dt * dt);
    const float cc = 2.0f * prm.self_damping_ratio * sqrtf(kk * mu);
    const float fn = kk * pen - cc * dot(vrel, n);
    if (fn <= 0.f) return false;
    const int32_t fx = (int32_t)rintf(n.x * fn * PHC_SC_FSCALE), fy = (int32_t)rintf(n.y * fn * PHC_SC_FSCALE), fz = (int32_t)rintf(n.z * fn * PHC_SC_FSCALE);
    const V3 F = v3((float)fx, (float)fy, (float)fz) * (1.0f / PHC_SC_FSCALE);
    const V3 ni = cross(cp - pi, F), nk = cross(cp - pk, F);
    int32_t* ai = reinterpret_cast<int32_t*>(caps + PHC_CAP_STRIDE * oi + 12);
    int32_t* ak = reinterpret_cast<int32_t*>(caps + PHC_CAP_STRIDE * ok + 12);
    sc_atomic_add(ai + 0, fx); sc_atomic_add(ai + 1, fy); sc_atomic_add(ai + 2, fz);
    sc_atomic_add(ak + 0, -fx); sc_atomic_add(ak + 1, -fy); sc_atomic_add(ak + 2, -fz);
    sc_atomic_add(ai + 3, (int32_t)rintf(ni.x * PHC_SC_NSCALE)); sc_atomic_add(ai + 4, (int32_t)rintf(ni.y * PHC_SC_NSCALE)); sc_atomic_add(ai + 5, (int32_t)rintf(ni.z * PHC_SC_NSCALE));
    sc_atomic_add(ak + 3, -(int32_t)rintf(nk.x * PHC_SC_NSCALE)); sc_atomic_add(ak + 4, -(int32_t)rintf(nk.y * PHC_SC_NSCALE)); sc_atomic_add(ak + 5, -(int32_t)rintf(nk.z * PHC_SC_NSCALE));
    return false;
}
PHC_HD bool aba_collide_pair(const phc_sim_params_t& prm, float dt, int i, int k, const Xch& x, float* caps) {
    const int b = aba_pair_broad(i, k, caps);
    return b == 0 ? aba_pair_narrow(prm, dt, i, k, x, caps) : b == 2;
}
#define PHC_SC_MAX_PER_LANE 18
template <int NP>
PHC_HD void aba_load_pairs(int* pr , int stride, const phc_model_t& m, int l, int nl) {
    const int np = model_num_pairs(m);
    int v[NP];
#if defined(__HIP_DEVICE_COMPILE__)
#pragma unroll
#endif
    for (int t = 0; t < NP; ++t) {
        const int q = t * nl + l;
        v[t] = m.ints[4 + PHC_NTAB * PHC_MAX_BODIES + (q < np ? 1 + q : 0)];
    }
#if defined(__HIP_DEVICE_COMPILE__)
#pragma unroll
#endif
    for (int t = 0; t < NP; ++t) pr[t * stride] = t * nl + l < np ? v[t] : -1;
}
template <int NP>
PHC_HD void aba_collide_pairs(const int* pr, int stride, const phc_sim_params_t& prm, float dt, const Xch& x, float* caps, uint32_t& near, bool refresh) {
    uint32_t cand = near, nr = 0u;
    if (refresh) {
        cand = 0u;
#if defined(__HIP_DEVICE_COMPILE__)
#pragma unroll
#endif
        for (int t = 0; t < NP; ++t) cand |= (pr[t * stride] >= 0 ? 1u : 0u) << t;
    }
    while (cand != 0u) {
        const int t = __builtin_ctz(cand);
        cand &= cand - 1u;
        const int pq = pr[t * stride];
        const int i = pq & 0xff, k = pq >> 8;
        const int b = aba_pair_broad(i, k, caps);
        const bool far = b == 0 ? aba_pair_narrow(prm, dt, i, k, x, caps) : b == 2;
        if (!far) nr |= 1u << t;
    }
    if (refresh) near = nr;
}
PHC_HD void aba_collect_self(AbaLane& L, int j, const float* caps) {
    const int32_t* acc = reinterpret_cast<const int32_t*>(caps + PHC_CAP_STRIDE * j + 12);
    L.fself = v3((float)acc[0], (float)acc[1], (float)acc[2]) * (1.0f / PHC_SC_FSCALE);
    L.nself = v3((float)acc[3], (float)acc[4], (float)acc[5]) * (1.0f / PHC_SC_NSCALE);
}

PHC_HD void shift_to_parent(const Inertia6& I, const Force6& p, V3 r, float* out , int es) {
    V3 c0 = v3(I.C.xx, I.C.xy, I.C.xz), c1 = v3(I.C.xy, I.C.yy, I.C.yz), c2 = v3(I.C.xz, I.C.yz, I.C.zz);
    V3 y0 = cross(r, c0), y1 = cross(r, c1), y2 = cross(r, c2);
    float Bp[9];
    Bp[0] = I.B[0] + y0.x; Bp[1] = I.B[1] + y1.x; Bp[2] = I.B[2] + y2.x;
    Bp[3] = I.B[3] + y0.y; Bp[4] = I.B[4] + y1.y; Bp[5] = I.B[5] + y2.y;
    Bp[6] = I.B[6] + y0.z; Bp[7] = I.B[7] + y1.z; Bp[8] = I.B[8] + y2.z;
    V3 b0 = v3(I.B[0], I.B[1], I.B[2]), b1 = v3(I.B[3], I.B[4], I.B[5]), b2 = v3(I.B[6], I.B[7], I.B[8]);
    V3 x0 = cross(r, b0), x1 = cross(r, b1), x2 = cross(r, b2);
    V3 bp0 = v3(Bp[0], Bp[1], Bp[2]), bp1 = v3(Bp[3], Bp[4], Bp[5]), bp2 = v3(Bp[6], Bp[7], Bp[8]);
    V3 z0 = cross(r, bp0), z1 = cross(r, bp1), z2 = cross(r, bp2);
    out[0 * es] = I.A.xx + x0.x + z0.x;
    out[1 * es] = I.A.xy + x0.y + z1.x;
    out[2 * es] = I.A.xz + x0.z + z2.x;
    out[3 * es] = I.A.yy + x1.y + z1.y;
    out[4 * es] = I.A.yz + x1.z + z2.y;
    out[5 * es] = I.A.zz + x2.z + z2.z;
    for (int k = 0; k < 9; ++k) out[(6 + k) * es] = Bp[k];
    out[15 * es] = I.C.xx; out[16 * es] = I.C.xy; out[17 * es] = I.C.xz; out[18 * es] = I.C.yy; out[19 * es] = I.C.yz; out[20 * es] = I.C.zz;
    V3 n = p.n + cross(r, p.f);
    out[21 * es] = n.x; out[22 * es] = n.y; out[23 * es] = n.z; out[24 * es] = p.f.x; out[25 * es] = p.f.y; out[26 * es] = p.f.z;
}

#define PHC_XCH_LAG 20
PHC_HD void xch_read6(const float* s, float* o) {
#if defined(__HIP_DEVICE_COMPILE__)
    const float4 a = *reinterpret_cast<const float4*>(s);
    const float2 b = *reinterpret_cast<const float2*>(s + 4);
    o[0] = a.x; o[1] = a.y; o[2] = a.z; o[3] = a.w; o[4] = b.x; o[5] = b.y;
#else
    for (int k = 0; k < 6; ++k) o[k] = s[k];
#endif
}
PHC_HD void xch_write6(float* s, const float* o) {
#if defined(__HIP_DEVICE_COMPILE__)
    *reinterpret_cast<float4*>(s) = make_float4(o[0], o[1], o[2], o[3]);
    *reinterpret_cast<float2*>(s + 4) = make_float2(o[4], o[5]);
#else
    for (int k = 0; k < 6; ++k) s[k] = o[k];
#endif
}

PHC_HD void accumulate_child(Inertia6& I, Force6& p, const float* s, int es) {
    I.A.xx += s[0 * es]; I.A.xy += s[1 * es]; I.A.xz += s[2 * es]; I.A.yy += s[3 * es]; I.A.yz += s[4 * es]; I.A.zz += s[5 * es];
    for (int k = 0; k < 9; ++k) I.B[k] += s[(6 + k) * es];
    I.C.xx += s[15 * es]; I.C.xy += s[16 * es]; I.C.xz += s[17 * es]; I.C.yy += s[18 * es]; I.C.yz += s[19 * es]; I.C.zz += s[20 * es];
    p.n.x += s[21 * es]; p.n.y += s[22 * es]; p.n.z += s[23 * es]; p.f.x += s[24 * es]; p.f.y += s[25 * es]; p.f.z += s[26 * es];
}

template <int JT>
PHC_HD void aba_backward_level(AbaLane& L, int level, int j, const Xch& x, bool lag = false) {
    if (L.slevel != level) return;
    if (lag) {
        constexpr int NB = aba_batched_constants<JT, false>() ? 3 : 1;
        float h[3][6];
        for (int k = 0; k < NB; ++k) xch_read6(xslot(x, k < L.nchild ? L.child[k] : j) + PHC_XCH_LAG, h[k]);
        for (int k = 0; k < 3; ++k) {
            const bool on = k < L.nchild;
            if (NB == 1 && k > 0) { if (!on) break; xch_read6(xslot(x, L.child[k]) + PHC_XCH_LAG, h[k]); }
            L.pA.n.x = on ? L.pA.n.x + h[k][0] : L.pA.n.x; L.pA.n.y = on ? L.pA.n.y + h[k][1] : L.pA.n.y; L.pA.n.z = on ? L.pA.n.z + h[k][2] : L.pA.n.z;
            L.pA.f.x = on ? L.pA.f.x + h[k][3] : L.pA.f.x; L.pA.f.y = on ? L.pA.f.y + h[k][4] : L.pA.f.y; L.pA.f.z = on ? L.pA.f.z + h[k][5] : L.pA.f.z;
        }
        if (level == 0) return;
        L.u = L.tau_w - L.pA.n;
        const V3 t = sym_mul(L.IA.A, L.cw) + B_mul(L.IA.B, L.ca);
        const V3 sb = Bt_mul(L.IA.B, L.cw) + sym_mul(L.IA.C, L.ca);
        const V3 z = sym_mul(L.Di, L.u - t);
        const V3 f = L.pA.f + sb + Bt_mul(L.IA.B, z);
        const V3 n = L.pA.n + t + sym_mul(L.IA.A, z) + cross(L.rw, f);
        const float o[6] = {n.x, n.y, n.z, f.x, f.y, f.z};
        xch_write6(xslot(x, j) + PHC_XCH_LAG, o);
        return;
    }
    for (int k = 0; k < 3; ++k)
        if (k < L.nchild) accumulate_child(L.IA, L.pA, xslot(x, L.child[k]), Xch::es);
    if (level == 0) return;
    if (JT == PHC_JT_REVOLUTE) {
        const V3 a = L.aw;
        const float ids = 1.0f / (dot(a, sym_mul(L.IA.A, a)) + L.dimp.x + L.arm.x);
        L.Di.xx = a.x * a.x * ids; L.Di.xy = a.x * a.y * ids; L.Di.xz = a.x * a.z * ids;
        L.Di.yy = a.y * a.y * ids; L.Di.yz = a.y * a.z * ids; L.Di.zz = a.z * a.z * ids;
    } else if (L.diso < 0.f) {
        Sym3 D = L.Dw;
        D.xx += L.IA.A.xx; D.xy += L.IA.A.xy; D.xz += L.IA.A.xz; D.yy += L.IA.A.yy; D.yz += L.IA.A.yz; D.zz += L.IA.A.zz;
        L.Di = sym_inv(D);
    }
    L.u = L.tau_w - L.pA.n;
    const Sym3& A = L.IA.A;
    const float* B = L.IA.B;
    V3 a0 = v3(A.xx, A.xy, A.xz), a1 = v3(A.xy, A.yy, A.yz), a2 = v3(A.xz, A.yz, A.zz);
    V3 bc0 = v3(B[0], B[3], B[6]), bc1 = v3(B[1], B[4], B[7]), bc2 = v3(B[2], B[5], B[8]);
    Inertia6 Ia;
    if (JT != PHC_JT_REVOLUTE && L.diso >= 0.f) {
        const float d = L.diso;
        Sym3 D = A;
        D.xx += d; D.yy += d; D.zz += d;
        L.Di = sym_inv(D);
        V3 p0 = v3(L.Di.xx, L.Di.xy, L.Di.xz), p1 = v3(L.Di.xy, L.Di.yy, L.Di.yz), p2 = v3(L.Di.xz, L.Di.yz, L.Di.zz);
        Ia.A.xx = d * dot(a0, p0); Ia.A.xy = d * dot(a0, p1); Ia.A.xz = d * dot(a0, p2);
        Ia.A.yy = d * dot(a1, p1); Ia.A.yz = d * dot(a1, p2); Ia.A.zz = d * dot(a2, p2);
        V3 h0 = sym_mul(L.Di, bc0), h1 = sym_mul(L.Di, bc1), h2 = sym_mul(L.Di, bc2);
        Ia.B[0] = d * h0.x; Ia.B[1] = d * h1.x; Ia.B[2] = d * h2.x;
        Ia.B[3] = d * h0.y; Ia.B[4] = d * h1.y; Ia.B[5] = d * h2.y;
        Ia.B[6] = d * h0.z; Ia.B[7] = d * h1.z; Ia.B[8] = d * h2.z;
        Ia.C.xx = L.IA.C.xx - dot(bc0, h0); Ia.C.xy = L.IA.C.xy - dot(bc0, h1); Ia.C.xz = L.IA.C.xz - dot(bc0, h2);
        Ia.C.yy = L.IA.C.yy - dot(bc1, h1); Ia.C.yz = L.IA.C.yz - dot(bc1, h2); Ia.C.zz = L.IA.C.zz - dot(bc2, h2);
    } else {
        V3 g0 = sym_mul(L.Di, a0), g1 = sym_mul(L.Di, a1), g2 = sym_mul(L.Di, a2);
        V3 h0 = sym_mul(L.Di, bc0), h1 = sym_mul(L.Di, bc1), h2 = sym_mul(L.Di, bc2);
        Ia.A.xx = A.xx - dot(a0, g0); Ia.A.xy = A.xy - dot(a0, g1); Ia.A.xz = A.xz - dot(a0, g2);
        Ia.A.yy = A.yy - dot(a1, g1); Ia.A.yz = A.yz - dot(a1, g2); Ia.A.zz = A.zz - dot(a2, g2);
        Ia.B[0] = B[0] - dot(a0, h0); Ia.B[1] = B[1] - dot(a0, h1); Ia.B[2] = B[2] - dot(a0, h2);
        Ia.B[3] = B[3] - dot(a1, h0); Ia.B[4] = B[4] - dot(a1, h1); Ia.B[5] = B[5] - dot(a1, h2);
        Ia.B[6] = B[6] - dot(a2, h0); Ia.B[7] = B[7] - dot(a2, h1); Ia.B[8] = B[8] - dot(a2, h2);
        Ia.C.xx = L.IA.C.xx - dot(bc0, h0); Ia.C.xy = L.IA.C.xy - dot(bc0, h1); Ia.C.xz = L.IA.C.xz - dot(bc0, h2);
        Ia.C.yy = L.IA.C.yy - dot(bc1, h1); Ia.C.yz = L.IA.C.yz - dot(bc1, h2); Ia.C.zz = L.IA.C.zz - dot(bc2, h2);
    }
    V3 du = sym_mul(L.Di, L.u);
    Force6 pa;
    pa.n = L.pA.n + sym_mul(Ia.A, L.cw) + B_mul(Ia.B, L.ca) + sym_mul(A, du);
    pa.f = L.pA.f + Bt_mul(Ia.B, L.cw) + sym_mul(Ia.C, L.ca) + Bt_mul(B, du);
    shift_to_parent(Ia, pa, L.rw, xslot(x, j), Xch::es);
}

template <int JT>
PHC_HD void aba_accel_level(AbaLane& L, int level, int j, const Xch& x) {
    if (L.slevel != level) return;
    constexpr int es = Xch::es;
    V3 alpha, a;
    if (level == 0) {
        Sym3 Ci = sym_inv(L.IA.C);
        const float* B = L.IA.B;
        V3 ci0 = v3(Ci.xx, Ci.xy, Ci.xz), ci1 = v3(Ci.xy, Ci.yy, Ci.yz), ci2 = v3(Ci.xz, Ci.yz, Ci.zz);
        V3 br0 = v3(B[0], B[1], B[2]), br1 = v3(B[3], B[4], B[5]), br2 = v3(B[6], B[7], B[8]);
        V3 w0 = v3(dot(br0, ci0), dot(br0, ci1), dot(br0, ci2));
        V3 w1 = v3(dot(br1, ci0), dot(br1, ci1), dot(br1, ci2));
        V3 w2 = v3(dot(br2, ci0), dot(br2, ci1), dot(br2, ci2));
        Sym3 S;
        S.xx = L.IA.A.xx - dot(w0, br0); S.xy = L.IA.A.xy - dot(w0, br1); S.xz = L.IA.A.xz - dot(w0, br2);
        S.yy = L.IA.A.yy - dot(w1, br1); S.yz = L.IA.A.yz - dot(w1, br2); S.zz = L.IA.A.zz - dot(w2, br2);
        V3 rhs = v3(-L.pA.n.x + dot(w0, L.pA.f), -L.pA.n.y + dot(w1, L.pA.f), -L.pA.n.z + dot(w2, L.pA.f));
        alpha = sym_mul(sym_inv(S), rhs);
        a = -sym_mul(Ci, L.pA.f + Bt_mul(B, alpha));
        L.u = alpha; L.ca = a;
        L.acc_w = alpha; L.acc_v = a;
    } else {
        const float* ps = xslot(x, L.sparent);
        V3 alp = v3(ps[0 * es], ps[1 * es], ps[2 * es]), ap = v3(ps[3 * es], ps[4 * es], ps[5 * es]);
        V3 al1 = alp + L.cw;
        V3 a1 = ap + cross(alp, L.rw) + L.ca;
        V3 beta = sym_mul(L.Di, L.u - sym_mul(L.IA.A, al1) - B_mul(L.IA.B, a1));
        alpha = al1 + beta;
        a = a1;
        L.u = beta;
        L.acc_w = alpha; L.acc_v = a;
    }
    float* s = xslot(x, j);
    s[0 * es] = alpha.x; s[1 * es] = alpha.y; s[2 * es] = alpha.z; s[3 * es] = a.x; s[4 * es] = a.y; s[5 * es] = a.z;
    s[19 * es] = L.u.x; s[20 * es] = L.u.y; s[21 * es] = L.u.z;
}

PHC_HD void aba_publish_drive(const AbaLane& L, int j, const Xch& x) {
    constexpr int es = Xch::es;
    float* s = xslot(x, j);
    s[19 * es] = L.tau_w.x; s[20 * es] = L.tau_w.y; s[21 * es] = L.tau_w.z;
    const bool iso = L.diso >= 0.f;
    s[22 * es] = iso ? L.diso : L.Dw.xx; s[23 * es] = iso ? 0.f : L.Dw.xy; s[24 * es] = iso ? 0.f : L.Dw.xz;
    s[25 * es] = iso ? L.diso : L.Dw.yy; s[26 * es] = iso ? 0.f : L.Dw.yz; s[27 * es] = iso ? L.diso : L.Dw.zz;
}
PHC_HD void aba_fetch_drive(AbaLane& L, int j, const Xch& x) {
    if (L.jsrc < 0 || L.jsrc == j) return;
    constexpr int es = Xch::es;
    const float* s = xslot(x, L.jsrc);
    L.tau_w = v3(-s[19 * es], -s[20 * es], -s[21 * es]);
    L.Dw.xx = s[22 * es]; L.Dw.xy = s[23 * es]; L.Dw.xz = s[24 * es]; L.Dw.yy = s[25 * es]; L.Dw.yz = s[26 * es]; L.Dw.zz = s[27 * es];
    const bool iso = L.Dw.xy == 0.f && L.Dw.xz == 0.f && L.Dw.yz == 0.f && L.Dw.xx == L.Dw.yy && L.Dw.yy == L.Dw.zz;
    L.diso = iso ? L.Dw.xx : -1.f;
}
PHC_HD void aba_accel_finish(AbaLane& L, const phc_model_t& m, int j, const Xch& x, const float* offs = nullptr ) {
    if (L.level < 0) return;
    constexpr int es = Xch::es;
    if (L.bsrc >= 0) {
        const float* s = xslot(x, L.bsrc);
        L.u = v3(-s[19 * es], -s[20 * es], -s[21 * es]);
    }
    if (L.level == 0 && L.slevel > 0) {
        const float* s = xslot(x, j);
        const float* f = offs ? offs + 3 * j : model_body(m, j) + 44;
        const V3 alpha = v3(s[0 * es], s[1 * es], s[2 * es]), a = v3(s[3 * es], s[4 * es], s[5 * es]);
        const V3 d = -quat_rotate(L.Q, v3(f[0], f[1], f[2]));
        L.u = alpha;
        L.ca = a + cross(alpha, d) + cross(L.w, cross(L.w, d));
    }
}

template <int JT>
PHC_HD void aba_integrate_joint(AbaLane& L, const phc_sim_params_t& prm, float dt) {
    if (L.level < 0) return;
    const float damp = 1.0f / (1.0f + dt * prm.angular_damping);
    if (L.level == 0) {
        const V3 alpha = L.u, a = L.ca;
        L.v = L.v + a * dt;
        L.w = (L.w + alpha * dt) * damp;
        L.p = L.p + L.v * dt;
        L.q = quat_normalize(quat_mul16(quat_from_rotvec(L.w * dt), L.q));
        return;
    }
    M3 R = quat_to_mat(L.Q);
    V3 qdd = mat_tmul(R, L.u);
    if (JT == PHC_JT_REVOLUTE) {
        const float thdd = dot(L.axis, qdd);
        L.tau_local = v3(dot(L.axis, L.tau_local) - L.dimp.x * thdd, 0.f, 0.f);
        L.thd = (L.thd + thdd * dt) * damp;
        L.thd = fminf(fmaxf(L.thd, -prm.max_angular_velocity), prm.max_angular_velocity);
        L.th += L.thd * dt;
        L.wj = L.axis * L.thd;
        L.q = rev_joint_quat(L);
    } else {
        L.tau_local = v3(L.tau_local.x - L.dimp.x * qdd.x, L.tau_local.y - L.dimp.y * qdd.y, L.tau_local.z - L.dimp.z * qdd.z);
        L.wj = (L.wj + qdd * dt) * damp;
        float wn = norm(L.wj);
        if (wn > prm.max_angular_velocity) L.wj = L.wj * (prm.max_angular_velocity / wn);
        L.q = quat_normalize(quat_mul16(L.q, quat_from_rotvec(L.wj * dt)));
    }
}

PHC_HD void aba_force_accumulate(AbaLane& L, int s, int n, float* acc ) {
    if (L.level < 0) return;
    V3 f = L.fcontact, t = L.tau_local;
    if (s > 0) { f += v3(acc[0], acc[1], acc[2]); t += v3(acc[3], acc[4], acc[5]); }
    if (s == n - 1) { const float w = 1.0f / (float)n; L.fcontact = f * w; L.tau_local = t * w; return; }
    acc[0] = f.x; acc[1] = f.y; acc[2] = f.z; acc[3] = t.x; acc[4] = t.y; acc[5] = t.z;
}

template <int JT>
PHC_HD void aba_store_state(const AbaLane& L, const phc_sim_state_t& s, int nd, int64_t env, int j) {
    if (j == 0) {
        float* r = s.root_states + env * 13;
        r[0] = L.p.x; r[1] = L.p.y; r[2] = L.p.z; r[3] = L.q.x; r[4] = L.q.y; r[5] = L.q.z; r[6] = L.q.w;
        r[7] = L.v.x; r[8] = L.v.y; r[9] = L.v.z; r[10] = L.w.x; r[11] = L.w.y; r[12] = L.w.z;
    } else if (JT == PHC_JT_REVOLUTE) {
        float* d = s.dof_state + (env * nd + L.dof_start) * 2;
        d[0] = L.th; d[1] = L.thd;
        if (s.dof_force) s.dof_force[env * nd + L.dof_start] = L.tau_local.x;
    } else {
        float* d = s.dof_state + (env * nd + L.dof_start) * 2;
        V3 e = quat_to_rotvec(L.q);
        d[0] = e.x; d[1] = L.wj.x; d[2] = e.y; d[3] = L.wj.y; d[4] = e.z; d[5] = L.wj.z;
        if (s.dof_force) {
            float* f = s.dof_force + env * nd + L.dof_start;
            f[0] = L.tau_local.x; f[1] = L.tau_local.y; f[2] = L.tau_local.z;
        }
    }
}
PHC_HD void aba_force_sensor(const AbaLane& L, const phc_model_t& m, const phc_sim_params_t& prm, float dt, int j, float* out6) {
    const float* f = model_body(m, j);
    const M3 R = quat_to_mat(L.Q);
    V3 F = v3(0.f, 0.f, 0.f), N = v3(0.f, 0.f, 0.f);
    const float cn = prm.contact_stiffness * dt + prm.contact_damping;
    const int cp_start = model_tab(m, 8, j), cp_total = model_tab(m, 9, j);
    const float* cp = m.floats + PHC_MAX_BODIES * PHC_BODY_FLOATS + cp_start * 4;
    const int cp_count = (L.p.z < f[34]) ? cp_total : 0;
    for (int k = 0; k < cp_count; ++k) {
        V3 arm = mat_mul(R, v3(cp[4 * k], cp[4 * k + 1], cp[4 * k + 2]));
        const float rad = cp[4 * k + 3];
        const float depth = rad - (L.p.z + arm.z);
        if (depth <= 0.f) continue;
        arm.z -= rad;
        const V3 uc = L.v + cross(L.w, arm);
        const float fn0 = prm.contact_stiffness * depth - cn * uc.z;
        if (fn0 <= 0.f) continue;
        const float ut = sqrtf(uc.x * uc.x + uc.y * uc.y);
        const float ct = fminf(prm.friction_viscous, prm.friction * fn0 / (ut + 1e-6f));
        const V3 F0 = v3(-ct * uc.x, -ct * uc.y, fn0);
        F += F0;
        N += cross(arm, F0);
    }
    const V3 Fl = mat_tmul(R, F), Nl = mat_tmul(R, N);
    out6[0] = Fl.x; out6[1] = Fl.y; out6[2] = Fl.z; out6[3] = Nl.x; out6[4] = Nl.y; out6[5] = Nl.z;
}
PHC_HD void aba_publish_sensors(const AbaLane& L, const phc_model_t& m, const phc_sim_params_t& prm, const phc_sim_state_t& s, float dt,
                                int64_t env, int j) {
    if (s.force_sensor == nullptr) return;
    for (int k = 0; k < prm.num_force_sensors; ++k)
        if (prm.force_sensor_body[k] == j) aba_force_sensor(L, m, prm, dt, j, s.force_sensor + (env * prm.num_force_sensors + k) * 6);
}

PHC_HD void aba_publish_body(const AbaLane& L, const phc_sim_state_t& s, int nb, int64_t env, int j, bool with_contact) {
    float* b = s.rigid_body_state + (env * nb + j) * 13;
    b[0] = L.p.x; b[1] = L.p.y; b[2] = L.p.z; b[3] = L.Q.x; b[4] = L.Q.y; b[5] = L.Q.z; b[6] = L.Q.w;
    b[7] = L.v.x; b[8] = L.v.y; b[9] = L.v.z; b[10] = L.w.x; b[11] = L.w.y; b[12] = L.w.z;
    if (with_contact && s.contact_force) {
        float* c = s.contact_force + (env * nb + j) * 3;
        c[0] = L.fcontact.x; c[1] = L.fcontact.y; c[2] = L.fcontact.z;
    }
}

}
```

### phc_amd/csrc/phc_sim.hip

```cpp
#include <hip/hip_runtime.h>
#include "phc_aba.h"

#ifdef PHC_SIM_PROFILE
__device__ unsigned long long g_phc_prof[16];
__device__ unsigned long long g_phc_prof_wg[8192][10];
__device__ unsigned long long g_phc_prof_where[8192][2];
extern "C" int32_t phc_debug_profile_wg(unsigned long long* out, int32_t nwg) {
    return hipMemcpyFromSymbol(out, HIP_SYMBOL(g_phc_prof_wg), sizeof(unsigned long long) * 10 * (nwg < 8192 ? nwg : 8192)) == hipSuccess ? 0 : -1;
}
extern "C" int32_t phc_debug_profile_where(unsigned long long* out, int32_t nwg) {
    return hipMemcpyFromSymbol(out, HIP_SYMBOL(g_phc_prof_where), sizeof(unsigned long long) * 2 * (nwg < 8192 ? nwg : 8192)) == hipSuccess ? 0 : -1;
}
extern "C" int32_t phc_debug_profile(unsigned long long* out16, int32_t reset) {
    if (out16 && hipMemcpyFromSymbol(out16, HIP_SYMBOL(g_phc_prof), sizeof(g_phc_prof)) != hipSuccess) return -1;
    if (reset) { unsigned long long z[16] = {0}; if (hipMemcpyToSymbol(HIP_SYMBOL(g_phc_prof), z, sizeof(z)) != hipSuccess) return -1; }
    return 0;
}
__device__ int g_phc_skip;
extern "C" int32_t phc_debug_set_skip(int32_t mask) { return hipMemcpyToSymbol(HIP_SYMBOL(g_phc_skip), &mask, sizeof(mask)) == hipSuccess ? 0 : -1; }
__device__ unsigned long long g_phc_tl[512];
__device__ int g_phc_tl_block = -1;
extern "C" int32_t phc_debug_timeline(unsigned long long* out512, int32_t block) {
    if (out512 && hipMemcpyFromSymbol(out512, HIP_SYMBOL(g_phc_tl), sizeof(g_phc_tl)) != hipSuccess) return -1;
    unsigned long long z[512] = {0};
    if (hipMemcpyToSymbol(HIP_SYMBOL(g_phc_tl), z, sizeof(z)) != hipSuccess) return -1;
    return hipMemcpyToSymbol(HIP_SYMBOL(g_phc_tl_block), &block, sizeof(block)) == hipSuccess ? 0 : -1;
}
#define PHC_TL_DECL int tl_n = 0; const bool tl_on = (int)blockIdx.x == g_phc_tl_block;
#define PHC_TL(id) if (tl_on && tl_sub == 1 && tl_n < 255) { __builtin_amdgcn_sched_barrier(0); const unsigned long long t_ = __builtin_readcyclecounter(); \
        if (threadIdx.x == 0) { g_phc_tl[2 * tl_n] = (unsigned long long)(id); g_phc_tl[2 * tl_n + 1] = t_; } ++tl_n; __builtin_amdgcn_sched_barrier(0); }
#define PHC_SKIP_DECL const int skip_mask = g_phc_skip;
#define PHC_SKIP(b) ((skip_mask >> (b)) & 1)
#define PHC_PROF_DECL unsigned long long prof_acc[10] = {0}; unsigned long long prof_t = __builtin_readcyclecounter(); const unsigned long long prof_t0 = prof_t; \
        const unsigned long long prof_hw = ((unsigned long long)__builtin_amdgcn_s_getreg((31 << 11) | 20) << 32) | (unsigned long long)__builtin_amdgcn_s_getreg((31 << 11) | 4);
#define PHC_PROF(i) if (!PHC_SKIP(15)) { __builtin_amdgcn_sched_barrier(0); __builtin_amdgcn_s_waitcnt(0); const unsigned long long t_ = __builtin_readcyclecounter(); prof_acc[i] += t_ - prof_t; prof_t = t_; __builtin_amdgcn_sched_barrier(0); }
#define PHC_PROF_FLUSH if (threadIdx.x == 0 && !PHC_SKIP(15)) { for (int i_ = 0; i_ < 10; ++i_) { atomicAdd(&g_phc_prof[i_], prof_acc[i_]); if (blockIdx.x < 8192) g_phc_prof_wg[blockIdx.x][i_] = prof_acc[i_]; } atomicAdd(&g_phc_prof[15], 1ull); \
        if (blockIdx.x < 8192) { g_phc_prof_where[blockIdx.x][0] = prof_t0; g_phc_prof_where[blockIdx.x][1] = prof_hw; } }
#endif

#include "phc_sim_kernel.h"
#include "phc_sim_check.h"

extern "C" {

int32_t phc_sim_step(const phc_model_t* model, const phc_sim_params_t* params, const phc_sim_state_t* sim, const float* actions,
                     const float* pd_action_offset, const float* pd_action_scale, const int32_t* freeze_mask,
                     int32_t num_sim_calls, void* stream) {
    int32_t rc = check_sim_step(model, params, sim, actions, pd_action_offset, pd_action_scale, num_sim_calls);
    if (rc || sim->num_envs == 0) return rc;
    sim_launch<true, false>(model, *params, sim, actions, pd_action_offset, pd_action_scale, freeze_mask, num_sim_calls, (hipStream_t)stream, nullptr, 0, WrenchArgs<false>());
    return launch_status();
}

int32_t phc_refresh_body_state(const phc_model_t* model, const phc_sim_state_t* sim, void* stream) {
    int32_t rc = check_model(model);
    if (rc) return rc;
    if (!sim || sim->num_envs < 0) return PHC_EINVAL;
    if (sim->num_envs == 0) return 0;
    phc_sim_params_t prm = {};
    prm.substeps = 1;
    sim_launch<false, false>(model, prm, sim, nullptr, nullptr, nullptr, nullptr, 0, (hipStream_t)stream, nullptr, 0, WrenchArgs<false>());
    return launch_status();
}

int32_t phc_refresh_body_state_indexed(const phc_model_t* model, const phc_sim_state_t* sim, int32_t num, const int64_t* env_ids,
                                       void* stream) {
    int32_t rc = check_model(model);
    if (rc) return rc;
    if (!sim || num < 0 || (num > 0 && !env_ids)) return PHC_EINVAL;
    if (num == 0) return 0;
    phc_sim_params_t prm = {};
    prm.substeps = 1;
    sim_launch<false, false>(model, prm, sim, nullptr, nullptr, nullptr, nullptr, 0, (hipStream_t)stream, env_ids, num, WrenchArgs<false>());
    return launch_status();
}

}
```

### phc_amd/csrc/phc_sim_kernel.h

```cpp
#pragma once
#include <hip/hip_runtime.h>
#include <type_traits>
#include "phc_aba.h"

using namespace phc;

#ifndef PHC_PROF_DECL
#define PHC_PROF_DECL
#define PHC_PROF(i)
#define PHC_PROF_FLUSH
#define PHC_SKIP_DECL
#define PHC_SKIP(b) false
#define PHC_TL_DECL
#define PHC_TL(id)
#endif

template <int K>
__device__ __forceinline__ void pd_targets_of(const phc_sim_state_t& sim, const float* __restrict__ actions, const float* __restrict__ pd_off,
                                              const float* __restrict__ pd_scale, const int32_t* __restrict__ freeze, const int32_t* valid_ints,
                                              int64_t env, int nd, int d0, float* tg) {
    const bool ref = sim.pd_ref != nullptr, frz = freeze != nullptr;
    const int64_t i0 = env * nd + d0;
    const float* basep = ref ? sim.pd_ref + i0 : pd_off + d0;
    const int32_t* frzp = frz ? freeze + d0 : valid_ints;
    float sc[K], ac[K], base[K], q[K];
    int32_t fz[K];
#pragma unroll
    for (int k = 0; k < K; ++k) {
        sc[k] = pd_scale[d0 + k]; ac[k] = actions[i0 + k]; base[k] = basep[k];
        q[k] = sim.dof_state[(i0 + k) * 2];
        fz[k] = frzp[k];
    }
#pragma unroll
    for (int k = 0; k < K; ++k) {
        float sa = __fmul_rn(sc[k], ac[k]);
        asm("" : "+v"(sa));
        const float half_pi = 1.57079637f;
        const float t0 = __fadd_rn(base[k], sa);
        const float t = ref ? fmaxf(fminf(t0, __fadd_rn(q[k], half_pi)), __fsub_rn(q[k], half_pi)) : t0;
        tg[k] = (frz && fz[k]) ? 0.f : t;
    }
}


struct StageLayout { int root, dof, force, contact, rbs, total; };
__device__ __forceinline__ StageLayout stage_layout(int E, int nb, int nd, bool with_force, bool with_contact) {
    StageLayout o;
    o.root = 0;
    o.dof = o.root + ((E * 13 + 3) & ~3);
    o.force = o.dof + ((E * nd * 2 + 3) & ~3);
    o.contact = o.force + (with_force ? ((E * nd + 3) & ~3) : 0);
    o.rbs = o.contact + (with_contact ? ((E * nb * 3 + 3) & ~3) : 0);
    o.total = o.rbs + ((E * nb * 13 + 3) & ~3);
    return o;
}
__device__ __forceinline__ phc_sim_state_t stage_state(const phc_sim_state_t& sim, float* stage, const StageLayout& o) {
    phc_sim_state_t st = sim;
    st.root_states = stage + o.root;
    st.dof_state = stage + o.dof;
    st.dof_force = sim.dof_force ? stage + o.force : nullptr;
    st.contact_force = sim.contact_force ? stage + o.contact : nullptr;
    st.rigid_body_state = stage + o.rbs;
    return st;
}
template <int W>
__device__ __forceinline__ void stage_copy_out(float* __restrict__ dst, const float* __restrict__ src, int n, int tid, int nthreads) {
    typedef typename std::conditional<W == 4, float4, float2>::type T;
    const int m = n / W;
    const T* s = reinterpret_cast<const T*>(src);
    T* d = reinterpret_cast<T*>(dst);
    int i = tid;
    for (; i + 3 * nthreads < m; i += 4 * nthreads) {
        const T a = s[i], b = s[i + nthreads], c = s[i + 2 * nthreads], e = s[i + 3 * nthreads];
        d[i] = a; d[i + nthreads] = b; d[i + 2 * nthreads] = c; d[i + 3 * nthreads] = e;
    }
    for (; i < m; i += nthreads) d[i] = s[i];
}
template <int E>
__device__ __forceinline__ void stage_flush(const phc_sim_state_t& sim, const float* stage, const StageLayout& o, int64_t env0, int nb, int nd) {
    constexpr int W = (E % 4 == 0) ? 4 : 2;
    const int tid = threadIdx.x;
    stage_copy_out<W>(sim.root_states + env0 * 13, stage + o.root, E * 13, tid, 64);
    stage_copy_out<W>(sim.dof_state + env0 * nd * 2, stage + o.dof, E * nd * 2, tid, 64);
    if (sim.dof_force) stage_copy_out<W>(sim.dof_force + env0 * nd, stage + o.force, E * nd, tid, 64);
    if (sim.contact_force) stage_copy_out<W>(sim.contact_force + env0 * nb * 3, stage + o.contact, E * nb * 3, tid, 64);
    stage_copy_out<W>(sim.rigid_body_state + env0 * nb * 13, stage + o.rbs, E * nb * 13, tid, 64);
}
__device__ __forceinline__ bool stage_aligned(const phc_sim_state_t& sim) {
    const uintptr_t a = (uintptr_t)sim.root_states | (uintptr_t)sim.dof_state | (uintptr_t)sim.rigid_body_state |
                        (uintptr_t)sim.dof_force | (uintptr_t)sim.contact_force;
    return (a & 15) == 0;
}

template <bool WRENCH> struct WrenchArgs {};
template <> struct WrenchArgs<true> { const float* force; const float* torque; int nsub; };

template <bool STEP, int JT, int GRP, bool SHAPES = false, bool RIGID = false, int OCC = 2, bool LAG = false, bool WRENCH = false>
__global__ __launch_bounds__(64, OCC) void k_sim_step(phc_model_t model_all, phc_sim_params_t prm, phc_sim_state_t sim,
                                                const float* __restrict__ actions, const float* __restrict__ pd_off,
                                                const float* __restrict__ pd_scale, const int32_t* __restrict__ freeze,
                                                int num_sim_calls, const int64_t* __restrict__ env_ids, int num_listed, WrenchArgs<WRENCH> wr) {
    __shared__ __attribute__((aligned(16))) float xch_all[64 * PHC_XCH_STRIDE];
    __shared__ float cap_all[64 * PHC_CAP_STRIDE];
    __shared__ int pair_all[PHC_SC_MAX_PER_LANE * 64];
    __shared__ float favg_all[STEP ? 64 * 6 : 1];
    constexpr bool BATCH = STEP && aba_batched_constants<JT, RIGID>();
    __shared__ float off_all[BATCH ? 64 * 3 : 1];
    constexpr bool WRENCH_TIGHT = WRENCH && LAG && JT == PHC_JT_REVOLUTE;
    const int lane = threadIdx.x & (GRP - 1);
    const int grp = threadIdx.x / GRP;
    const int64_t slot = (int64_t)blockIdx.x * (64 / GRP) + grp;
    const int64_t env = (!STEP && env_ids != nullptr) ? (slot < num_listed ? env_ids[slot] : sim.num_envs) : slot;
    const phc_model_t model = SHAPES ? model_for_env(model_all, sim, env) : model_all;
    const int nb = model.num_bodies, nd = model.num_dof;
    const bool active = env < sim.num_envs && lane < nb;
    const int body = lane;
    Xch x;
    x.base = xch_all + grp * GRP * PHC_XCH_STRIDE;

    AbaLane L;
    L.level = L.slevel = -1;
    PHC_SKIP_DECL
    PHC_PROF_DECL
    PHC_TL_DECL
    if (active) {
        aba_load_model(L, model, body);
        if (JT == PHC_JT_REVOLUTE) aba_load_model_rev(L, model, body);
        if (BATCH) { const float* f = model_body(model, body); float* o = off_all + grp * GRP * 3 + body * 3; o[0] = f[44]; o[1] = f[45]; o[2] = f[46]; }
        const bool new_targets = STEP && actions != nullptr && body >= 1;
        aba_load_state<JT>(L, sim, nd, env, body, !new_targets);
        if (new_targets) {
            constexpr int K = JT == PHC_JT_REVOLUTE ? 1 : 3;
            float tg[3] = {0.f, 0.f, 0.f};
            pd_targets_of<K>(sim, actions, pd_off, pd_scale, freeze, model.ints, env, nd, L.dof_start, tg);
#pragma unroll
            for (int k = 0; k < K; ++k) sim.pd_target[env * nd + L.dof_start + k] = tg[k];
            L.target = v3(tg[0], tg[1], tg[2]);
        }
    }
    const bool shape_lane = active || (STEP && prm.self_collision && env < sim.num_envs && lane < nb + model_num_extra_shapes(model));
    if (shape_lane && !active) aba_load_extra_shape(L, model, lane - nb);
    if (!PHC_SKIP(8)) {
        const int jsteps = model_jump_steps(model);
        aba_fk_jump_begin(L, body, x);
        __syncthreads();
        for (int k = 0; k < jsteps; ++k) {
            aba_fk_jump_step(L, k, x);
            __syncthreads();
            if (active) aba_write_kin(L, xslot(x, body), Xch::es, 6);
            __syncthreads();
        }
    }
    PHC_PROF(0)
    if (STEP) {
        const float dt = prm.sim_dt / (float)prm.substeps;
        const int nsub = num_sim_calls * prm.substeps;
        float* caps = cap_all + grp * GRP * PHC_CAP_STRIDE;
        const float* offs = BATCH ? off_all + grp * GRP * 3 : nullptr;
        uint32_t near_pairs = 0;
        if (prm.self_collision) aba_load_pairs<PHC_SC_MAX_PER_LANE>(pair_all + threadIdx.x, 64, model, lane, GRP);
        const int solver_depth = model_solver_depth(model, true);
        const int jump_steps = model_jump_steps(model);
        const bool rerooted = model_tab(model, 11, 3) != 0;
        for (int s = 0; s < nsub; ++s) {
            const int tl_sub = s; (void)tl_sub;
            PHC_TL(1)
            V3 ext_f = v3(0.f, 0.f, 0.f), ext_t = v3(0.f, 0.f, 0.f);
            bool ext_on = false;
            if constexpr (WRENCH) {
                ext_on = s < wr.nsub;
                if (ext_on && active) {
                    const int64_t wi = (env * nb + body) * 3;
                    if (wr.force != nullptr) ext_f = v3(wr.force[wi], wr.force[wi + 1], wr.force[wi + 2]);
                    if (wr.torque != nullptr) ext_t = v3(wr.torque[wi], wr.torque[wi + 1], wr.torque[wi + 2]);
                }
            }
            if (prm.self_collision && !PHC_SKIP(0)) {
                if (shape_lane) aba_publish_shape(L, lane, x, caps);
                __syncthreads();
                if (env < sim.num_envs) aba_collide_pairs<PHC_SC_MAX_PER_LANE>(pair_all + threadIdx.x, 64, prm, dt, x, caps, near_pairs, s == 0);
                __syncthreads();
                if (active) aba_collect_self(L, body, caps);
            }
            PHC_PROF(1)
            PHC_TL(2)
            if (active && !PHC_SKIP(1)) aba_velocity_products(L, model, body, x, true, offs);
            const int passes = RIGID ? (prm.contact_iterations < 1 ? 1 : prm.contact_iterations) : 1;
            const bool lag = LAG && !RIGID && (s % prm.substeps) != 0;
            for (int pass = 0; pass < passes; ++pass) {
            PHC_TL(3)
            if (active && !PHC_SKIP(1)) {
                if constexpr (WRENCH) {
                    float dt_b = dt;
                    if constexpr (WRENCH_TIGHT) asm volatile("" : "+v"(dt_b));
                    if (!BATCH) aba_body_init<JT, RIGID>(L, model, prm, dt_b, body, s % prm.substeps == 0, true, pass, lag, ext_on, ext_f, ext_t);
                    else aba_body_init<JT, RIGID>(L, model, prm, dt_b, body, s % prm.substeps == 0, model_body(model, body), L.cp_range & 0xffff, L.cp_range >> 16, true, pass, lag,
                                                  ext_on, ext_f, ext_t);
                } else {
                if (!BATCH) aba_body_init<JT, RIGID>(L, model, prm, dt, body, s % prm.substeps == 0, true, pass, lag);
                else aba_body_init<JT, RIGID>(L, model, prm, dt, body, s % prm.substeps == 0, model_body(model, body), L.cp_range & 0xffff, L.cp_range >> 16, true, pass, lag);
                }
            }
            if (active && PHC_SKIP(9)) aba_body_init<JT, RIGID>(L, model, prm, dt, body, s % prm.substeps == 0, true, pass, lag);
            PHC_PROF(2)
            PHC_TL(4)
            if (JT == PHC_JT_SPHERICAL && rerooted && pass == 0 && !PHC_SKIP(2)) {
                if (active) aba_publish_drive(L, body, x);
                __syncthreads();
                if (active) aba_fetch_drive(L, body, x);
                __syncthreads();
            }
            PHC_PROF(3)
            PHC_TL(5)
            if (!PHC_SKIP(3)) for (int l = solver_depth; l >= 0; --l) { aba_backward_level<JT>(L, l, body, x, lag); __syncthreads(); PHC_TL(120 + l) }
            PHC_PROF(4)
            if (!PHC_SKIP(4)) {
                for (int l = 0; l <= solver_depth; ++l) { aba_accel_level<JT>(L, l, body, x); __syncthreads(); PHC_TL(140 + l) }
            }
            }
            if (RIGID && active && (s == nsub - 1 || prm.force_average)) aba_publish_contact_rigid(L, model, prm, sim, dt, env, body, true);
            if (JT == PHC_JT_SPHERICAL && rerooted && !PHC_SKIP(4)) aba_accel_finish(L, model, body, x, offs);
            PHC_PROF(5)
            PHC_TL(6)
            if (!PHC_SKIP(5)) aba_integrate_joint<JT>(L, prm, dt);
            if (prm.force_average) aba_force_accumulate(L, s, nsub, favg_all + threadIdx.x * 6);
            PHC_PROF(6)
            PHC_TL(7)
            if (!PHC_SKIP(6)) aba_fk_jump_begin(L, body, x);
            __syncthreads();
            for (int k = 0; k < (PHC_SKIP(6) ? 0 : jump_steps); ++k) {
                aba_fk_jump_step(L, k, x);
                __syncthreads();
                if (active) aba_write_kin(L, xslot(x, body), Xch::es, 6);
                __syncthreads();
                PHC_TL(160 + k)
            }
            PHC_PROF(7)
            PHC_TL(8)
        }
    }
    constexpr int E = 64 / GRP;
    const int64_t env0 = (int64_t)blockIdx.x * E;
    const StageLayout so = stage_layout(E, nb, nd, sim.dof_force != nullptr, sim.contact_force != nullptr);
    if (PHC_SKIP(7)) {
    } else if (STEP && E >= 2 && env0 + E <= sim.num_envs && stage_aligned(sim) && so.total <= 64 * PHC_XCH_STRIDE) {
        const phc_sim_state_t st = stage_state(sim, xch_all, so);
        if (active) {
            aba_store_state<JT>(L, st, nd, grp, body);
            aba_publish_body(L, st, nb, grp, body, true);
        }
        __syncthreads();
        stage_flush<E>(sim, xch_all, so, env0, nb, nd);
    } else if (active) {
        if (STEP) aba_store_state<JT>(L, sim, nd, env, body);
        aba_publish_body(L, sim, nb, env, body, STEP);
    }
    if (STEP && !RIGID && active && sim.force_sensor != nullptr) aba_publish_sensors(L, model, prm, sim, prm.sim_dt / (float)prm.substeps, env, body);
    PHC_PROF(8)
    if (STEP) { PHC_PROF_FLUSH }
}

template <bool STEP, int JT, bool SHAPES, bool RIGID, bool WRENCH>
static void sim_launch_cm(const phc_model_t* model, const phc_sim_params_t& prm, const phc_sim_state_t* sim, const float* actions, const float* off,
                          const float* scale, const int32_t* freeze, int num_sim_calls, hipStream_t stream, const int64_t* env_ids, int num_listed,
                          const WrenchArgs<WRENCH>& wr) {
    const int64_t groups = env_ids ? num_listed : sim->num_envs;
    const bool wide = model->num_bodies > 32;
    constexpr bool LAG = STEP && !RIGID;
    const bool lag = LAG && prm.inertia_lag != 0;
    auto launch = [&](auto kernel, int64_t blocks) {
        hipLaunchKernelGGL(kernel, dim3(blocks), dim3(64), 0, stream, *model, prm, *sim, actions, off, scale, freeze, num_sim_calls, env_ids, num_listed, wr);
    };
    if constexpr (!WRENCH && LAG && !SHAPES && JT == PHC_JT_SPHERICAL)
        if (!wide && prm.lane_mapping == 3) return launch(k_sim_step<STEP, JT, 32, SHAPES, RIGID, 3>, (groups + 1) / 2);
    if (lag && wide) launch(k_sim_step<STEP, JT, 64, SHAPES, RIGID, 2, LAG, WRENCH>, groups);
    else if (lag) launch(k_sim_step<STEP, JT, 32, SHAPES, RIGID, 2, LAG, WRENCH>, (groups + 1) / 2);
    else if (wide) launch(k_sim_step<STEP, JT, 64, SHAPES, RIGID, 2, false, WRENCH>, groups);
    else launch(k_sim_step<STEP, JT, 32, SHAPES, RIGID, 2, false, WRENCH>, (groups + 1) / 2);
}

template <bool STEP, int JT, bool SHAPES, bool WRENCH>
static void sim_launch_jt(const phc_model_t* model, const phc_sim_params_t& prm, const phc_sim_state_t* sim, const float* actions, const float* off,
                          const float* scale, const int32_t* freeze, int num_sim_calls, hipStream_t stream, const int64_t* env_ids, int num_listed,
                          const WrenchArgs<WRENCH>& wr) {
    if (STEP && prm.contact_model == 1)
        sim_launch_cm<STEP, JT, SHAPES, STEP, WRENCH>(model, prm, sim, actions, off, scale, freeze, num_sim_calls, stream, env_ids, num_listed, wr);
    else
        sim_launch_cm<STEP, JT, SHAPES, false, WRENCH>(model, prm, sim, actions, off, scale, freeze, num_sim_calls, stream, env_ids, num_listed, wr);
}
template <bool STEP, bool WRENCH>
static void sim_launch(const phc_model_t* model, const phc_sim_params_t& prm, const phc_sim_state_t* sim, const float* actions, const float* off,
                       const float* scale, const int32_t* freeze, int num_sim_calls, hipStream_t stream, const int64_t* env_ids, int num_listed,
                       const WrenchArgs<WRENCH>& wr) {
    if (model->num_dof == model->num_bodies - 1 && model->num_bodies > 2)
        return sim_launch_jt<STEP, PHC_JT_REVOLUTE, false, WRENCH>(model, prm, sim, actions, off, scale, freeze, num_sim_calls, stream, env_ids, num_listed, wr);
    if constexpr (!WRENCH)
        if (model->num_shapes > 1 && sim->env_shape != nullptr)
            return sim_launch_jt<STEP, PHC_JT_SPHERICAL, true, false>(model, prm, sim, actions, off, scale, freeze, num_sim_calls, stream, env_ids, num_listed, wr);
    sim_launch_jt<STEP, PHC_JT_SPHERICAL, false, WRENCH>(model, prm, sim, actions, off, scale, freeze, num_sim_calls, stream, env_ids, num_listed, wr);
}

static inline int32_t launch_status() {
    hipError_t e = hipGetLastError();
    return e == hipSuccess ? 0 : (int32_t)e;
}
```

Before: 40.25 million.

## Add specialized plain sim-step kernel with pinned model constants and isotropic drives

```diff
diff --git a/include/phc_amd.h b/include/phc_amd.h
--- a/include/phc_amd.h
+++ b/include/phc_amd.h
@@ -25,7 +25,9 @@
     int32_t int_stride;
     int32_t float_stride;
     int32_t max_body_contact_pts;
+    int32_t sim_plain_facts;
 } phc_model_t;
+#define PHC_SIM_FACTS_PLAIN 0x504c4e01
 
 typedef struct {
     const float* frames;
@@ -187,6 +189,11 @@
                             const int32_t* freeze_mask , int32_t num_sim_calls,
                             const float* ext_force , const float* ext_torque , int32_t wrench_sim_calls, void* stream);
 
+int32_t phc_sim_model_facts(const phc_model_t* model_on_host);
+int32_t phc_sim_is_plain(const phc_model_t* model, const phc_sim_params_t* params, const phc_sim_state_t* sim, const float* actions,
+                         const int32_t* freeze_mask, int32_t num_sim_calls);
+int32_t phc_sim_force_generic(int32_t on);
+
 int32_t phc_refresh_body_state(const phc_model_t* model, const phc_sim_state_t* sim, void* stream);
 
 int32_t phc_refresh_body_state_indexed(const phc_model_t* model, const phc_sim_state_t* sim, int32_t num, const int64_t* env_ids,
diff --git a/phc_amd/_lib.py b/phc_amd/_lib.py
--- a/phc_amd/_lib.py
+++ b/phc_amd/_lib.py
@@ -15,7 +15,7 @@
 class Model(C.Structure):
     _fields_ = [("num_bodies", c_i32), ("num_dof", c_i32), ("max_level", c_i32), ("num_contact_pts", c_i32),
                 ("ints", c_p), ("floats", c_p), ("num_collision_pairs", c_i32),
-                ("num_shapes", c_i32), ("int_stride", c_i32), ("float_stride", c_i32), ("max_body_contact_pts", c_i32)]
+                ("num_shapes", c_i32), ("int_stride", c_i32), ("float_stride", c_i32), ("max_body_contact_pts", c_i32), ("sim_plain_facts", c_i32)]
 
 
 class MotionLib(C.Structure):
@@ -158,6 +158,9 @@
 _OPTIONAL_SIGNATURES = {
     "phc_im_is_plain": ([P(Model), P(MotionLib), P(ImParams), P(ImBuffers)], c_i32),
     "phc_task_force_generic": ([c_i32], c_i32),
+    "phc_sim_model_facts": ([P(Model)], c_i32),
+    "phc_sim_is_plain": ([P(Model), P(SimParams), P(SimState), c_p, c_p, c_i32], c_i32),
+    "phc_sim_force_generic": ([c_i32], c_i32),
 }
 EXPORTED_SYMBOLS = tuple(_SIGNATURES) + tuple(_OPTIONAL_SIGNATURES)
 
diff --git a/phc_amd/abi.py b/phc_amd/abi.py
--- a/phc_amd/abi.py
+++ b/phc_amd/abi.py
@@ -31,7 +31,21 @@
     per_body = ints.reshape(max(1, int(num_shapes)), -1)[:, 4 + 9 * MAX_BODIES:4 + 10 * MAX_BODIES]
     m.max_body_contact_pts = int(per_body.max())
     m.ints, m.floats = ptr(ints), ptr(floats)
+    m.sim_plain_facts = _sim_plain_facts(m, ints, floats)
     return m
+
+
+def _sim_plain_facts(m, ints, floats):
+    fn = getattr(L.load(), "phc_sim_model_facts", None)
+    if fn is None or m.num_shapes > 1:
+        return 0
+    hi, hf = (np.ascontiguousarray(t if isinstance(t, np.ndarray) else t.detach().cpu().numpy()) for t in (ints, floats))
+    if hi.dtype != np.int32 or hf.dtype != np.float32:
+        return 0
+    h = L.Model()
+    C.memmove(C.byref(h), C.byref(m), C.sizeof(m))
+    h.ints, h.floats = hi.ctypes.data, hf.ctypes.data
+    return int(fn(C.byref(h)))
 
 
 def motion_lib_struct(frames, frame_stride, num_bodies, motion_lengths, motion_dt, motion_num_frames, length_starts,
diff --git a/phc_amd/build.py b/phc_amd/build.py
--- a/phc_amd/build.py
+++ b/phc_amd/build.py
@@ -7,10 +7,10 @@
 CSRC = os.path.join(HERE, "csrc")
 LIB = os.path.join(HERE, "libphc_amd.so")
 SOURCES = {"phc_kernels.hip": ["-fno-slp-vectorize", "-ffp-contract=off"], "phc_kernels_plain.hip": ["-fno-slp-vectorize", "-ffp-contract=off"], "phc_sim.hip": ["-ffast-math", "-fno-slp-vectorize"],
-           "phc_sim_wrench.hip": ["-ffast-math", "-fno-slp-vectorize"],
+           "phc_sim_wrench.hip": ["-ffast-math", "-fno-slp-vectorize"], "phc_sim_plain.hip": ["-ffast-math", "-fno-slp-vectorize"],
            "phc_learn.hip": ["-ffp-contract=off"], "phc_gemm.hip": ["-ffp-contract=off"], "phc_render.hip": [], "phc_eval.hip": ["-ffp-contract=off"],
            "phc_push.hip": ["-ffp-contract=off"]}
-HEADERS = ["phc_math.h", "phc_task.h", "phc_im.h", "phc_im_check.h", "phc_im_plain.h", "phc_task_kernel.h", "phc_aba.h", "phc_sim_kernel.h", "phc_sim_check.h", "phc_eval.h", "phc_group.h", "phc_rng.h", "phc_push.h", os.path.join("..", "..", "include", "phc_amd.h")]
+HEADERS = ["phc_math.h", "phc_task.h", "phc_im.h", "phc_im_check.h", "phc_im_plain.h", "phc_task_kernel.h", "phc_aba.h", "phc_sim_kernel.h", "phc_sim_check.h", "phc_sim_plain.h", "phc_eval.h", "phc_group.h", "phc_rng.h", "phc_push.h", os.path.join("..", "..", "include", "phc_amd.h")]
 
 
 def _hipcc():
diff --git a/phc_amd/csrc/phc_aba.h b/phc_amd/csrc/phc_aba.h
--- a/phc_amd/csrc/phc_aba.h
+++ b/phc_amd/csrc/phc_aba.h
@@ -382,15 +382,25 @@
     L.pA.n -= T + cross(mc, F) * (1.0f / mass);
 }
 
-template <int JT, bool RIGID>
+#define ABA_PL_NO_CP_TAIL 1
+#define ABA_PL_DRIVE_CONST 2
+struct AbaPlainDrive { float kp, kdp; V3 eff; };
+PHC_HD void aba_plain_drive(AbaLane& L, AbaPlainDrive& pd, const float* f, float dt) {
+    const float kp = f[13], kd = f[16];
+    pd.kp = kp; pd.kdp = kd + dt * kp; pd.eff = v3(f[22], f[23], f[24]);
+    const float d = dt * kd + dt * dt * kp;
+    L.dimp = v3(d, d, d);
+    L.diso = d + f[19];
+}
+template <int JT, bool RIGID, int PL = 0>
 PHC_HD void aba_body_init(AbaLane& L, const phc_model_t& m, const phc_sim_params_t& prm, float dt, int j, bool new_sim_call,
                           const float* f, int cp_start, int cp_total, bool reroot, int pass, bool lag = false,
-                          bool ext_on = false, V3 ext_f = V3(), V3 ext_t = V3()) {
+                          bool ext_on = false, V3 ext_f = V3(), V3 ext_t = V3(), const AbaPlainDrive* pd = nullptr) {
     constexpr bool BATCH = aba_batched_constants<JT, RIGID>();
     const float mass = BATCH ? L.mass : f[3];
     const SolverRef sr = model_solver_ref(f, reroot);
     float fd[12];
-    if (BATCH) for (int k = 0; k < 12; ++k) fd[k] = f[13 + k];
+    if (BATCH && !(PL & ABA_PL_DRIVE_CONST)) for (int k = 0; k < 12; ++k) fd[k] = f[13 + k];
     M3 R = quat_to_mat(L.Q);
     const float* cp = m.floats + PHC_MAX_BODIES * PHC_BODY_FLOATS + cp_start * 4;
     int cp_count = 0;
@@ -461,6 +471,7 @@
         }
     }
     if (!lag) {
+        if (!(PL & ABA_PL_NO_CP_TAIL))
         for (int k = PHC_CP_BITS; k < cp_count; ++k) cp_point(cp_load(k));
         L.c_touch = pushed;
     }
@@ -513,6 +524,15 @@
     if (L.level > 0) {
         Q4 qt = quat_from_rotvec(L.target);
         V3 err = quat_to_rotvec(quat_mul16(quat_conjugate(L.q), qt));
+        if (PL & ABA_PL_DRIVE_CONST) {
+            const float kp = pd->kp, kdp = pd->kdp;
+            const V3 eff = pd->eff;
+            const V3 tau = v3(fminf(fmaxf(kp * err.x, -eff.x), eff.x) - kdp * L.wj.x, fminf(fmaxf(kp * err.y, -eff.y), eff.y) - kdp * L.wj.y,
+                              fminf(fmaxf(kp * err.z, -eff.z), eff.z) - kdp * L.wj.z);
+            L.tau_local = tau;
+            L.tau_w = mat_mul(R, tau);
+            return;
+        }
         const float* fg = BATCH ? fd : f + 13;
         const V3 kp = v3(fg[0], fg[1], fg[2]), kd = v3(fg[3], fg[4], fg[5]), eff = v3(fg[9], fg[10], fg[11]);
         V3 sp = v3(fminf(fmaxf(kp.x * err.x, -eff.x), eff.x), fminf(fmaxf(kp.y * err.y, -eff.y), eff.y), fminf(fmaxf(kp.z * err.z, -eff.z), eff.z));
@@ -746,7 +766,7 @@
     p.n.x += s[21 * es]; p.n.y += s[22 * es]; p.n.z += s[23 * es]; p.f.x += s[24 * es]; p.f.y += s[25 * es]; p.f.z += s[26 * es];
 }
 
-template <int JT>
+template <int JT, bool ISO = false>
 PHC_HD void aba_backward_level(AbaLane& L, int level, int j, const Xch& x, bool lag = false) {
     if (L.slevel != level) return;
     if (lag) {
@@ -778,7 +798,7 @@
         const float ids = 1.0f / (dot(a, sym_mul(L.IA.A, a)) + L.dimp.x + L.arm.x);
         L.Di.xx = a.x * a.x * ids; L.Di.xy = a.x * a.y * ids; L.Di.xz = a.x * a.z * ids;
         L.Di.yy = a.y * a.y * ids; L.Di.yz = a.y * a.z * ids; L.Di.zz = a.z * a.z * ids;
-    } else if (L.diso < 0.f) {
+    } else if (!ISO && L.diso < 0.f) {
         Sym3 D = L.Dw;
         D.xx += L.IA.A.xx; D.xy += L.IA.A.xy; D.xz += L.IA.A.xz; D.yy += L.IA.A.yy; D.yz += L.IA.A.yz; D.zz += L.IA.A.zz;
         L.Di = sym_inv(D);
@@ -789,7 +809,7 @@
     V3 a0 = v3(A.xx, A.xy, A.xz), a1 = v3(A.xy, A.yy, A.yz), a2 = v3(A.xz, A.yz, A.zz);
     V3 bc0 = v3(B[0], B[3], B[6]), bc1 = v3(B[1], B[4], B[7]), bc2 = v3(B[2], B[5], B[8]);
     Inertia6 Ia;
-    if (JT != PHC_JT_REVOLUTE && L.diso >= 0.f) {
+    if (JT != PHC_JT_REVOLUTE && (ISO || L.diso >= 0.f)) {
         const float d = L.diso;
         Sym3 D = A;
         D.xx += d; D.yy += d; D.zz += d;
@@ -858,22 +878,29 @@
     s[19 * es] = L.u.x; s[20 * es] = L.u.y; s[21 * es] = L.u.z;
 }
 
-PHC_HD void aba_publish_drive(const AbaLane& L, int j, const Xch& x) {
+PHC_HD void aba_publish_drive(const AbaLane& L, int j, const Xch& x, bool tau_only = false) {
     constexpr int es = Xch::es;
     float* s = xslot(x, j);
     s[19 * es] = L.tau_w.x; s[20 * es] = L.tau_w.y; s[21 * es] = L.tau_w.z;
+    if (tau_only) return;
     const bool iso = L.diso >= 0.f;
     s[22 * es] = iso ? L.diso : L.Dw.xx; s[23 * es] = iso ? 0.f : L.Dw.xy; s[24 * es] = iso ? 0.f : L.Dw.xz;
     s[25 * es] = iso ? L.diso : L.Dw.yy; s[26 * es] = iso ? 0.f : L.Dw.yz; s[27 * es] = iso ? L.diso : L.Dw.zz;
 }
-PHC_HD void aba_fetch_drive(AbaLane& L, int j, const Xch& x) {
+PHC_HD void aba_fetch_drive(AbaLane& L, int j, const Xch& x, bool tau_only = false) {
     if (L.jsrc < 0 || L.jsrc == j) return;
     constexpr int es = Xch::es;
     const float* s = xslot(x, L.jsrc);
     L.tau_w = v3(-s[19 * es], -s[20 * es], -s[21 * es]);
+    if (tau_only) return;
     L.Dw.xx = s[22 * es]; L.Dw.xy = s[23 * es]; L.Dw.xz = s[24 * es]; L.Dw.yy = s[25 * es]; L.Dw.yz = s[26 * es]; L.Dw.zz = s[27 * es];
     const bool iso = L.Dw.xy == 0.f && L.Dw.xz == 0.f && L.Dw.yz == 0.f && L.Dw.xx == L.Dw.yy && L.Dw.yy == L.Dw.zz;
     L.diso = iso ? L.Dw.xx : -1.f;
+}
+PHC_HD void aba_publish_diso(const AbaLane& L, int j, const Xch& x) { xslot(x, j)[22 * Xch::es] = L.diso; }
+PHC_HD void aba_fetch_diso(AbaLane& L, int j, const Xch& x) {
+    if (L.jsrc < 0 || L.jsrc == j) return;
+    L.diso = xslot(x, L.jsrc)[22 * Xch::es];
 }
 PHC_HD void aba_accel_finish(AbaLane& L, const phc_model_t& m, int j, const Xch& x, const float* offs = nullptr ) {
     if (L.level < 0) return;
diff --git a/phc_amd/csrc/phc_sim.hip b/phc_amd/csrc/phc_sim.hip
--- a/phc_amd/csrc/phc_sim.hip
+++ b/phc_amd/csrc/phc_sim.hip
@@ -41,7 +41,26 @@
 #include "phc_sim_kernel.h"
 #include "phc_sim_check.h"
 
+#ifdef PHC_SIM_PROFILE
+int32_t g_phc_sim_force_generic = 1;
+#else
+int32_t g_phc_sim_force_generic = 0;
+#endif
+
 extern "C" {
+
+int32_t phc_sim_force_generic(int32_t on) {
+    const int32_t old = g_phc_sim_force_generic;
+    g_phc_sim_force_generic = on ? 1 : 0;
+    return old;
+}
+
+int32_t phc_sim_model_facts(const phc_model_t* model_on_host) { return sim_model_facts(model_on_host); }
+
+int32_t phc_sim_is_plain(const phc_model_t* model, const phc_sim_params_t* params, const phc_sim_state_t* sim, const float* actions, const int32_t* freeze_mask,
+                         int32_t num_sim_calls) {
+    return sim_is_plain(model, params, sim, actions, freeze_mask, num_sim_calls) ? 1 : 0;
+}
 
 int32_t phc_sim_step(const phc_model_t* model, const phc_sim_params_t* params, const phc_sim_state_t* sim, const float* actions,
                      const float* pd_action_offset, const float* pd_action_scale, const int32_t* freeze_mask,
diff --git a/phc_amd/csrc/phc_sim_kernel.h b/phc_amd/csrc/phc_sim_kernel.h
--- a/phc_amd/csrc/phc_sim_kernel.h
+++ b/phc_amd/csrc/phc_sim_kernel.h
@@ -2,6 +2,7 @@
 #include <hip/hip_runtime.h>
 #include <type_traits>
 #include "phc_aba.h"
+#include "phc_sim_plain.h"
 
 using namespace phc;
 
@@ -92,10 +93,34 @@
     return (a & 15) == 0;
 }
 
+#define SIM_PL_LAG_PAIR 8
+#ifndef PHC_SIM_PLAIN_ITEMS
+#define PHC_SIM_PLAIN_ITEMS (ABA_PL_NO_CP_TAIL | ABA_PL_DRIVE_CONST | SIM_PL_LAG_PAIR)
+#endif
+template <bool PLAIN>
+__device__ __forceinline__ void pin_sim_plain(phc_sim_params_t& prm, phc_sim_state_t& sim, const float* __restrict__& actions, const int32_t* __restrict__& freeze,
+                                              int& num_sim_calls) {
+    if constexpr (PLAIN) {
+#define PHC_PIN_prm(f) prm.f
+#define PHC_PIN_sim(f) sim.f
+#define PHC_PIN_arg(f) f
+#define PHC_PIN_VAL(s, f, v) PHC_PIN_##s(f) = (v);
+#define PHC_PIN_NUL(s, f) PHC_PIN_##s(f) = nullptr;
+#define PHC_PIN_SET(s, f) __builtin_assume(PHC_PIN_##s(f) != nullptr);
+        PHC_SIM_PLAIN_FIELDS(PHC_PIN_VAL, PHC_PIN_NUL, PHC_PIN_SET)
+#undef PHC_PIN_VAL
+#undef PHC_PIN_NUL
+#undef PHC_PIN_SET
+#undef PHC_PIN_prm
+#undef PHC_PIN_sim
+#undef PHC_PIN_arg
+    }
+}
+
 template <bool WRENCH> struct WrenchArgs {};
 template <> struct WrenchArgs<true> { const float* force; const float* torque; int nsub; };
 
-template <bool STEP, int JT, int GRP, bool SHAPES = false, bool RIGID = false, int OCC = 2, bool LAG = false, bool WRENCH = false>
+template <bool STEP, int JT, int GRP, bool SHAPES = false, bool RIGID = false, int OCC = 2, bool LAG = false, bool WRENCH = false, bool PLAIN = false>
 __global__ __launch_bounds__(64, OCC) void k_sim_step(phc_model_t model_all, phc_sim_params_t prm, phc_sim_state_t sim,
                                                 const float* __restrict__ actions, const float* __restrict__ pd_off,
                                                 const float* __restrict__ pd_scale, const int32_t* __restrict__ freeze,
@@ -107,12 +132,15 @@
     constexpr bool BATCH = STEP && aba_batched_constants<JT, RIGID>();
     __shared__ float off_all[BATCH ? 64 * 3 : 1];
     constexpr bool WRENCH_TIGHT = WRENCH && LAG && JT == PHC_JT_REVOLUTE;
+    static_assert(!PLAIN || (STEP && JT == PHC_JT_SPHERICAL && GRP == 32 && !SHAPES && !RIGID && OCC == 2 && LAG && !WRENCH), "the one plain instantiation");
+    constexpr int PL = PLAIN ? (PHC_SIM_PLAIN_ITEMS) : 0;
+    pin_sim_plain<PLAIN>(prm, sim, actions, freeze, num_sim_calls);
     const int lane = threadIdx.x & (GRP - 1);
     const int grp = threadIdx.x / GRP;
     const int64_t slot = (int64_t)blockIdx.x * (64 / GRP) + grp;
     const int64_t env = (!STEP && env_ids != nullptr) ? (slot < num_listed ? env_ids[slot] : sim.num_envs) : slot;
     const phc_model_t model = SHAPES ? model_for_env(model_all, sim, env) : model_all;
-    const int nb = model.num_bodies, nd = model.num_dof;
+    const int nb = PLAIN ? SimPlainModel::num_bodies : model.num_bodies, nd = PLAIN ? SimPlainModel::num_dof : model.num_dof;
     const bool active = env < sim.num_envs && lane < nb;
     const int body = lane;
     Xch x;
@@ -138,10 +166,10 @@
             L.target = v3(tg[0], tg[1], tg[2]);
         }
     }
-    const bool shape_lane = active || (STEP && prm.self_collision && env < sim.num_envs && lane < nb + model_num_extra_shapes(model));
+    const bool shape_lane = active || (STEP && prm.self_collision && env < sim.num_envs && lane < nb + (PLAIN ? SimPlainModel::extra_shapes : model_num_extra_shapes(model)));
     if (shape_lane && !active) aba_load_extra_shape(L, model, lane - nb);
     if (!PHC_SKIP(8)) {
-        const int jsteps = model_jump_steps(model);
+        const int jsteps = PLAIN ? SimPlainModel::jump_steps : model_jump_steps(model);
         aba_fk_jump_begin(L, body, x);
         __syncthreads();
         for (int k = 0; k < jsteps; ++k) {
@@ -159,9 +187,19 @@
         const float* offs = BATCH ? off_all + grp * GRP * 3 : nullptr;
         uint32_t near_pairs = 0;
         if (prm.self_collision) aba_load_pairs<PHC_SC_MAX_PER_LANE>(pair_all + threadIdx.x, 64, model, lane, GRP);
-        const int solver_depth = model_solver_depth(model, true);
-        const int jump_steps = model_jump_steps(model);
-        const bool rerooted = model_tab(model, 11, 3) != 0;
+        const int solver_depth = PLAIN ? SimPlainModel::solver_depth : model_solver_depth(model, true);
+        const int jump_steps = PLAIN ? SimPlainModel::jump_steps : model_jump_steps(model);
+        const bool rerooted = PLAIN ? SimPlainModel::rerooted != 0 : model_tab(model, 11, 3) != 0;
+        constexpr int SUBSTEP_UNROLL = (PL & SIM_PL_LAG_PAIR) ? 2 : 1;
+        AbaPlainDrive pdrive;
+        if constexpr ((PL & ABA_PL_DRIVE_CONST) != 0) {
+            if (active && L.level > 0) aba_plain_drive(L, pdrive, model_body(model, body), dt);
+            if (active) { if (L.level == 0) L.diso = 0.f; aba_publish_diso(L, body, x); }
+            __syncthreads();
+            if (active) aba_fetch_diso(L, body, x);
+            __syncthreads();
+        }
+#pragma unroll SUBSTEP_UNROLL
         for (int s = 0; s < nsub; ++s) {
             const int tl_sub = s; (void)tl_sub;
             PHC_TL(1)
@@ -196,6 +234,9 @@
                     if (!BATCH) aba_body_init<JT, RIGID>(L, model, prm, dt_b, body, s % prm.substeps == 0, true, pass, lag, ext_on, ext_f, ext_t);
                     else aba_body_init<JT, RIGID>(L, model, prm, dt_b, body, s % prm.substeps == 0, model_body(model, body), L.cp_range & 0xffff, L.cp_range >> 16, true, pass, lag,
                                                   ext_on, ext_f, ext_t);
+                } else if constexpr (PLAIN) {
+                    aba_body_init<JT, RIGID, PL>(L, model, prm, dt, body, s % prm.substeps == 0, model_body(model, body), L.cp_range & 0xffff, L.cp_range >> 16, true, pass, lag,
+                                                 false, V3(), V3(), &pdrive);
                 } else {
                 if (!BATCH) aba_body_init<JT, RIGID>(L, model, prm, dt, body, s % prm.substeps == 0, true, pass, lag);
                 else aba_body_init<JT, RIGID>(L, model, prm, dt, body, s % prm.substeps == 0, model_body(model, body), L.cp_range & 0xffff, L.cp_range >> 16, true, pass, lag);
@@ -205,14 +246,14 @@
             PHC_PROF(2)
             PHC_TL(4)
             if (JT == PHC_JT_SPHERICAL && rerooted && pass == 0 && !PHC_SKIP(2)) {
-                if (active) aba_publish_drive(L, body, x);
-                __syncthreads();
-                if (active) aba_fetch_drive(L, body, x);
+                if (active) aba_publish_drive(L, body, x, (PL & ABA_PL_DRIVE_CONST) != 0);
+                __syncthreads();
+                if (active) aba_fetch_drive(L, body, x, (PL & ABA_PL_DRIVE_CONST) != 0);
                 __syncthreads();
             }
             PHC_PROF(3)
             PHC_TL(5)
-            if (!PHC_SKIP(3)) for (int l = solver_depth; l >= 0; --l) { aba_backward_level<JT>(L, l, body, x, lag); __syncthreads(); PHC_TL(120 + l) }
+            if (!PHC_SKIP(3)) for (int l = solver_depth; l >= 0; --l) { aba_backward_level<JT, (PL & ABA_PL_DRIVE_CONST) != 0>(L, l, body, x, lag); __syncthreads(); PHC_TL(120 + l) }
             PHC_PROF(4)
             if (!PHC_SKIP(4)) {
                 for (int l = 0; l <= solver_depth; ++l) { aba_accel_level<JT>(L, l, body, x); __syncthreads(); PHC_TL(140 + l) }
@@ -243,7 +284,7 @@
     const int64_t env0 = (int64_t)blockIdx.x * E;
     const StageLayout so = stage_layout(E, nb, nd, sim.dof_force != nullptr, sim.contact_force != nullptr);
     if (PHC_SKIP(7)) {
-    } else if (STEP && E >= 2 && env0 + E <= sim.num_envs && stage_aligned(sim) && so.total <= 64 * PHC_XCH_STRIDE) {
+    } else if (STEP && E >= 2 && env0 + E <= sim.num_envs && (PLAIN || stage_aligned(sim)) && so.total <= 64 * PHC_XCH_STRIDE) {
         const phc_sim_state_t st = stage_state(sim, xch_all, so);
         if (active) {
             aba_store_state<JT>(L, st, nd, grp, body);
@@ -259,6 +300,12 @@
     PHC_PROF(8)
     if (STEP) { PHC_PROF_FLUSH }
 }
+
+extern int32_t g_phc_sim_force_generic;
+extern template __global__ void k_sim_step<true, PHC_JT_SPHERICAL, 32, false, false, 2, true, false, true>(phc_model_t, phc_sim_params_t, phc_sim_state_t, const float* __restrict__,
+                                                                                                           const float* __restrict__, const float* __restrict__,
+                                                                                                           const int32_t* __restrict__, int, const int64_t* __restrict__, int,
+                                                                                                           WrenchArgs<false>);
 
 template <bool STEP, int JT, bool SHAPES, bool RIGID, bool WRENCH>
 static void sim_launch_cm(const phc_model_t* model, const phc_sim_params_t& prm, const phc_sim_state_t* sim, const float* actions, const float* off,
@@ -273,6 +320,9 @@
     };
     if constexpr (!WRENCH && LAG && !SHAPES && JT == PHC_JT_SPHERICAL)
         if (!wide && prm.lane_mapping == 3) return launch(k_sim_step<STEP, JT, 32, SHAPES, RIGID, 3>, (groups + 1) / 2);
+    if constexpr (STEP && !WRENCH && LAG && !SHAPES && JT == PHC_JT_SPHERICAL)
+        if (lag && !wide && !g_phc_sim_force_generic && sim_is_plain(model, &prm, sim, actions, freeze, num_sim_calls))
+            return launch(k_sim_step<true, PHC_JT_SPHERICAL, 32, false, false, 2, true, false, true>, (groups + 1) / 2);
     if (lag && wide) launch(k_sim_step<STEP, JT, 64, SHAPES, RIGID, 2, LAG, WRENCH>, groups);
     else if (lag) launch(k_sim_step<STEP, JT, 32, SHAPES, RIGID, 2, LAG, WRENCH>, (groups + 1) / 2);
     else if (wide) launch(k_sim_step<STEP, JT, 64, SHAPES, RIGID, 2, false, WRENCH>, groups);
diff --git a/phc_amd/csrc/phc_sim_plain.h b/phc_amd/csrc/phc_sim_plain.h
--- /dev/null
+++ b/phc_amd/csrc/phc_sim_plain.h
@@ -0,0 +1,85 @@
+#pragma once
+#include "phc_aba.h"
+
+#define PHC_SIM_PLAIN_FIELDS(VAL, NUL, SET) \
+    VAL(prm, substeps, 2) \
+    VAL(prm, control_mode, 0) \
+    VAL(prm, self_collision, 1) \
+    VAL(prm, lane_mapping, 0) \
+    VAL(prm, contact_model, 0) \
+    VAL(prm, inertia_lag, 1) \
+    VAL(arg, num_sim_calls, 2) \
+    SET(arg, actions) \
+    SET(arg, freeze) \
+    NUL(sim, force_sensor) \
+    NUL(sim, env_shape) \
+    NUL(sim, pd_ref) \
+    SET(sim, contact_force) \
+    SET(sim, dof_force)
+
+#define PHC_SIM_PLAIN_MODEL(FACT) \
+    FACT(num_bodies, 24) \
+    FACT(num_dof, 69) \
+    FACT(solver_depth, 6) \
+    FACT(jump_steps, 4) \
+    FACT(rerooted, 1) \
+    FACT(extra_shapes, 2)
+
+#define PHC_SIM_PLAIN_CP_MAX 32
+
+namespace phc {
+
+struct SimPlainArgs { const float* actions; const int32_t* freeze; int32_t num_sim_calls; };
+
+PHC_HD int sim_fact_num_bodies(const phc_model_t& m) { return m.num_bodies; }
+PHC_HD int sim_fact_num_dof(const phc_model_t& m) { return m.num_dof; }
+PHC_HD int sim_fact_solver_depth(const phc_model_t& m) { return model_solver_depth(m, true); }
+PHC_HD int sim_fact_jump_steps(const phc_model_t& m) { return model_jump_steps(m); }
+PHC_HD int sim_fact_rerooted(const phc_model_t& m) { return model_tab(m, 11, 3) != 0 ? 1 : 0; }
+PHC_HD int sim_fact_extra_shapes(const phc_model_t& m) { return model_num_extra_shapes(m); }
+
+constexpr int sim_plain_pad4(int n) { return (n + 3) & ~3; }
+struct SimPlainModel {
+#define PHC_PLAIN_FACT(n, v) static constexpr int n = (v);
+    PHC_SIM_PLAIN_MODEL(PHC_PLAIN_FACT)
+#undef PHC_PLAIN_FACT
+    static constexpr int stage_total = sim_plain_pad4(2 * 13) + sim_plain_pad4(2 * num_dof * 2) + sim_plain_pad4(2 * num_dof) + sim_plain_pad4(2 * num_bodies * 3) + sim_plain_pad4(2 * num_bodies * 13);
+};
+static_assert(SimPlainModel::stage_total <= 64 * PHC_XCH_STRIDE, "the plain kernel takes the staged epilogue unconditionally: it must fit the exchange area");
+static_assert(SimPlainModel::num_bodies + SimPlainModel::extra_shapes <= 32 && SimPlainModel::num_dof == 3 * (SimPlainModel::num_bodies - 1), "spherical joints, 32 lanes per env");
+
+inline int32_t sim_model_facts(const phc_model_t* m) {
+    if (!m || !m->ints || !m->floats || m->num_bodies < 1 || m->num_bodies > 32 || m->num_shapes > 1) return 0;
+#define PHC_PLAIN_FACT(n, v) if (sim_fact_##n(*m) != (v)) return 0;
+    PHC_SIM_PLAIN_MODEL(PHC_PLAIN_FACT)
+#undef PHC_PLAIN_FACT
+    if (m->max_body_contact_pts > PHC_SIM_PLAIN_CP_MAX) return 0;
+    for (int j = 0; j < m->num_bodies; ++j) {
+        if (model_tab(*m, 9, j) > PHC_SIM_PLAIN_CP_MAX) return 0;
+        if (j > 0 && model_tab(*m, 2, j) != PHC_JT_SPHERICAL) return 0;
+        const float* f = model_body(*m, j);
+        for (int o = 13; j > 0 && o < 22; o += 3) if (f[o] != f[o + 1] || f[o] != f[o + 2]) return 0;
+    }
+    return PHC_SIM_FACTS_PLAIN;
+}
+
+inline bool sim_is_plain(const phc_model_t* model, const phc_sim_params_t* prm, const phc_sim_state_t* sim, const float* actions, const int32_t* freeze,
+                         int32_t num_sim_calls) {
+    if (!model || !prm || !sim) return false;
+    if (model->sim_plain_facts != PHC_SIM_FACTS_PLAIN || model->num_shapes > 1 || model->max_body_contact_pts > PHC_SIM_PLAIN_CP_MAX) return false;
+    if (model->num_bodies != SimPlainModel::num_bodies || model->num_dof != SimPlainModel::num_dof) return false;
+    const SimPlainArgs args = {actions, freeze, num_sim_calls};
+    const SimPlainArgs* arg = &args;
+#define PHC_PLAIN_VAL(s, f, v) if (s->f != (v)) return false;
+#define PHC_PLAIN_NUL(s, f) if (s->f != nullptr) return false;
+#define PHC_PLAIN_SET(s, f) if (s->f == nullptr) return false;
+    PHC_SIM_PLAIN_FIELDS(PHC_PLAIN_VAL, PHC_PLAIN_NUL, PHC_PLAIN_SET)
+#undef PHC_PLAIN_VAL
+#undef PHC_PLAIN_NUL
+#undef PHC_PLAIN_SET
+    const uintptr_t a = (uintptr_t)sim->root_states | (uintptr_t)sim->dof_state | (uintptr_t)sim->rigid_body_state | (uintptr_t)sim->dof_force |
+                        (uintptr_t)sim->contact_force;
+    return (a & 15) == 0;
+}
+
+}
diff --git a/phc_amd/csrc/phc_sim_plain.hip b/phc_amd/csrc/phc_sim_plain.hip
--- /dev/null
+++ b/phc_amd/csrc/phc_sim_plain.hip
@@ -0,0 +1,6 @@
+#include "phc_sim_kernel.h"
+
+template __global__ void k_sim_step<true, PHC_JT_SPHERICAL, 32, false, false, 2, true, false, true>(phc_model_t, phc_sim_params_t, phc_sim_state_t, const float* __restrict__,
+                                                                                                    const float* __restrict__, const float* __restrict__,
+                                                                                                    const int32_t* __restrict__, int, const int64_t* __restrict__, int,
+                                                                                                    WrenchArgs<false>);
```

Result: faster. 42.20 million, median of 6 (+4.8%).
